# undistro/trivy

Hardware: AMD Instinct MI355X
Metric: GB/s secret-scanned (whole node) at 1/2/4/8 MI355X; findings bit-exact vs CPU (higher is better)
Workload: dtype u8

## Files before the change

include/tsg_debug.h:

```cpp
#ifndef TSG_DEBUG_H
#define TSG_DEBUG_H
#include <stdint.h>
#ifdef __cplusplus
extern "C" {
#endif

int tsg_regex_find_all(const char* pattern, const uint8_t* text, uint64_t n, int submatch,
                       const int64_t* windows, uint32_t n_windows, int64_t* out, uint64_t out_cap,
                       uint64_t* out_len, int32_t* num_cap);

void tsg_debug_regex_engine(int mode);
int tsg_debug_xform(int device, const uint8_t* raw, uint64_t n_bytes, const uint64_t* offsets, uint32_t n_files,
                    const uint8_t* kinds, uint8_t* out, uint64_t out_cap, uint64_t* xoff);
int tsg_debug_classify(int device, const uint8_t* raw, uint64_t n_bytes, const uint64_t* offsets, uint32_t n_files,
                       uint8_t* flags);
int tsg_debug_transform_census(int device, const uint8_t* raw, uint64_t n_bytes, const uint64_t* offsets,
                               uint32_t n_files, const uint8_t* kinds, uint8_t* mark_out);
int tsg_debug_gather_device(int device, const uint8_t* raw, uint64_t n_bytes, const uint64_t* src_off,
                            const uint64_t* dst_off, uint32_t n_files, uint8_t* out);
int tsg_regex_match(const char* pattern, const uint8_t* text, uint64_t n);

int64_t tsg_go_bytes_to_lower(const uint8_t* s, uint64_t n, uint8_t* out, uint64_t out_cap);

struct tsg_global;
typedef struct tsg_compiled tsg_compiled;
struct tsg_table_info;
typedef struct tsg_debug_rule_info {
  uint32_t nfa_words;
  uint32_t gate;
  uint32_t anchored;
  uint32_t has_regex;
  const uint64_t* nfa;
  const uint32_t* kw_ids;
  uint32_t n_kw;
} tsg_debug_rule_info;
int tsg_debug_compile(const struct tsg_global* g, tsg_compiled** out);
struct tsg_compile_options;
int tsg_debug_compile_ex(const struct tsg_global* g, const struct tsg_compile_options* opt, tsg_compiled** out,
                         uint32_t* out_calibrated);
void tsg_debug_compiled_free(tsg_compiled* c);
int tsg_debug_compiled_info(const tsg_compiled* c, struct tsg_table_info* out);
int tsg_debug_rule(const tsg_compiled* c, uint32_t i, tsg_debug_rule_info* out);
int tsg_debug_rule_gate_implied(const tsg_compiled* c, uint32_t i);
int tsg_debug_anchor(const tsg_compiled* c, uint32_t j, uint32_t* rule, uint32_t* lit_len,
                     int32_t* off_lo, int32_t* off_hi);
const char* tsg_debug_keyword(const tsg_compiled* c, uint32_t k);
const void* tsg_debug_anchor_req(const tsg_compiled* c, uint32_t j);
int tsg_debug_filter(const tsg_compiled* c, uint32_t* shape, const uint32_t** reach, const uint32_t** bucket_off,
                     const uint32_t** bucket_items, const void** items, uint32_t* n_items, const uint8_t** item_cls,
                     const uint32_t** classes, double* est_fp);
int tsg_debug_filter_ids(const tsg_compiled* c, const uint32_t** ids, uint32_t* n);
int tsg_debug_filter_core(const tsg_compiled* c, uint32_t out[4]);
const char* tsg_debug_rule_anchor(const tsg_compiled* c, uint32_t i);


int tsg_debug_pool_budget(void);

struct tsg_scanner;
int tsg_debug_scanner_engine(struct tsg_scanner* s, uint64_t out[4]);
int tsg_debug_filter_orform(const tsg_compiled* c, uint32_t out[1024]);

int tsg_debug_scanner_gpu_findings(struct tsg_scanner* s, int mode);

int tsg_debug_scanner_fetch(struct tsg_scanner* s, uint64_t stage_bytes, uint64_t direct_bytes);

int tsg_regex_find_all_bounded(const char* pattern, const uint8_t* text, uint64_t true_len, uint64_t lo, uint64_t hi,
                               int submatch, const int64_t* windows, uint32_t n_windows, int64_t* out,
                               uint64_t out_cap, uint64_t* out_len, int32_t* num_cap, int32_t* hit_limit);
int tsg_debug_fetch_windows_plan(const uint64_t* offsets, uint32_t n_files, const void* cands, uint64_t n_cands,
                                 const uint32_t* rule_max_len, uint32_t n_rules, const uint32_t* opts, uint64_t* runs,
                                 uint64_t runs_cap, uint64_t* n_runs, uint64_t* views, uint64_t views_cap,
                                 uint64_t* n_views, uint64_t totals[4]);
int tsg_debug_fetch_windows_device(int device, const uint8_t* arena, uint64_t n_bytes, const uint64_t* offsets,
                                   uint32_t n_files, const void* cands, uint64_t n_cands, uint32_t cand_cap,
                                   const uint32_t* rule_max_len, uint32_t n_rules, const uint32_t* opts,
                                   uint64_t stage_bytes, uint8_t* packed, uint64_t packed_cap, uint64_t counters[4]);

struct tsg_batch;
struct tsg_result;
struct tsg_fetch_window_stats;
int tsg_debug_sparse_tail(const struct tsg_global* g, const struct tsg_batch* batch, const void* cands,
                          uint64_t n_cands, const uint32_t* opts, struct tsg_result** out,
                          struct tsg_fetch_window_stats* window_stats);

int tsg_debug_sure_allow(const char* const* patterns, uint32_t n_patterns, const uint8_t* paths, const uint64_t* off,
                         uint32_t n_paths, uint8_t* sure, uint8_t* has_form);
int tsg_debug_result_skip(const struct tsg_result* r, uint64_t out[6]);
int tsg_debug_result_k0(const struct tsg_result* r, double* ms_k0);

typedef struct tsg_debug_stage_dump {
  uint32_t struct_size;
  uint32_t kw_words;
  uint32_t counters[16];
  uint32_t caps[3];
  uint32_t reserved_;
  uint64_t* hits;        uint64_t hits_cap, n_hits;
  uint32_t* kw;          uint64_t kw_cap, n_kw;
  uint32_t* flags;       uint64_t flags_cap, n_flags;
  uint16_t* nl;          uint64_t nl_cap, n_nl;
  uint32_t* chunk_file;  uint64_t chunk_file_cap, n_chunk_file;
  uint32_t* recs;        uint64_t recs_cap, n_recs;
  void* cands;           uint64_t cands_cap, n_cands;
} tsg_debug_stage_dump;
int tsg_debug_engine_stages(const tsg_compiled* c, int device, const uint8_t* arena, uint64_t n_bytes,
                            const uint64_t* offsets, uint32_t n_files, const uint8_t tail[64],
                            tsg_debug_stage_dump* out);
int tsg_debug_engine_stages_skip(const tsg_compiled* c, int device, const uint8_t* arena, uint64_t n_bytes,
                                 const uint64_t* offsets, uint32_t n_files, const uint8_t tail[64],
                                 const uint8_t* skip, tsg_debug_stage_dump* out);
int tsg_debug_scan_grow(const uint32_t counters[16], const uint32_t fs_counters[6], uint32_t caps[7]);

int tsg_debug_tar_headers(int device, const void* dev_tar, uint64_t n_bytes, uint64_t capacity, uint32_t grid_cap,
                          void* records_out, uint64_t* count_out, double* ms_out);
void tsg_debug_set_tar_capacity(uint64_t records);
struct tsg_analyzer;
struct tsg_tar_index;
struct tsg_device_tar_stats;
int tsg_debug_index_tar_records(struct tsg_analyzer* a, const uint8_t* host_tar, uint64_t n_bytes,
                                const void* records, uint64_t n_records, struct tsg_tar_index** out,
                                struct tsg_device_tar_stats* st);
int tsg_debug_tar_chain(int device, const void* dev_tar, uint64_t n_bytes, uint32_t segment_blocks, uint32_t grid_cap,
                        void* records_out, uint64_t rec_cap, uint64_t* n_records, uint8_t* names_out,
                        uint64_t name_cap, uint64_t* name_bytes, uint64_t* stop_out, uint64_t* candidates_out);
int tsg_debug_tar_walk_last_fallback(const struct tsg_analyzer* a);
int tsg_debug_index_tar_entries(struct tsg_analyzer* a, const void* records, uint64_t n_records, const uint8_t* names,
                                uint64_t name_bytes, const uint64_t* stop, uint64_t n_bytes,
                                uint64_t candidates_given, struct tsg_tar_index** out,
                                struct tsg_device_tar_stats* st);
int tsg_debug_tar_batch_plan(const struct tsg_tar_index* ix, uint32_t first, uint32_t count, const uint8_t* flags,
                             uint64_t* base, uint64_t* offs, uint8_t* kinds, uint8_t* binary);

const char* tsg_last_error(void);

#ifdef __cplusplus
}
#endif
#endif
```

trivy_amd/csrc/capi_debug.cpp:

```cpp
#include "tsg_debug.h"

#include <algorithm>
#include <atomic>
#include <cstring>
#include <memory>
#include <string>
#include <vector>

#include "capi_internal.h"
#include "census.h"
#include "classify.h"
#include "fetch_host.h"
#include "fetch_windows.h"
#include "filter.h"
#include "goregex.h"
#include "k1_orform.h"
#include "parallel.h"
#include "xform.h"

namespace tsg {
extern std::atomic<int> g_regex_engine;
thread_local std::string g_last_error;
void SetError(const std::string& e) { g_last_error = e; }
}
// ... 439 lines not shown

int tsg_debug_engine_stages(const tsg_compiled* c, int device, const uint8_t* arena, uint64_t n_bytes,
                            const uint64_t* offsets, uint32_t n_files, const uint8_t tail[64],
                            tsg_debug_stage_dump* out) {
  return tsg_debug_engine_stages_skip(c, device, arena, n_bytes, offsets, n_files, tail, nullptr, out);
}

int tsg_debug_engine_stages_skip(const tsg_compiled* c, int device, const uint8_t* arena, uint64_t n_bytes,
                                 const uint64_t* offsets, uint32_t n_files, const uint8_t tail[64],
                                 const uint8_t* skip, tsg_debug_stage_dump* out) {
  if (!c || !offsets || !tail || !out || (n_bytes && !arena)) {
    tsg::SetError("tsg_debug_engine_stages: NULL argument");
    return -2;
  }
  if (out->struct_size != sizeof(tsg_debug_stage_dump)) {
    tsg::SetError("tsg_debug_engine_stages: unknown tsg_debug_stage_dump.struct_size");
    return -2;
  }
  if (!WinArgsOk("tsg_debug_engine_stages", offsets, n_files, nullptr)) return -2;
  if (offsets[n_files] != n_bytes) {
    tsg::SetError("tsg_debug_engine_stages: offsets must end at n_bytes");
    return -2;
  }
  void *d_arena = nullptr, *d_off = nullptr, *d_skip = nullptr;
  hipError_t e = hipSetDevice(device);
  auto ok = [&](hipError_t r) {
    if (e == hipSuccess) e = r;
    return e == hipSuccess;
  };
  tsg::StageDump d;
  std::string run_err;
  if (ok(e) && ok(hipMalloc(&d_arena, n_bytes + 64)) && ok(hipMalloc(&d_off, (size_t(n_files) + 1) * 8)) &&
      ok(hipMemcpy(static_cast<uint8_t*>(d_arena) + n_bytes, tail, 64, hipMemcpyHostToDevice)) &&
      (n_bytes == 0 || ok(hipMemcpy(d_arena, arena, n_bytes, hipMemcpyHostToDevice))) &&
      ok(hipMemcpy(d_off, offsets, (size_t(n_files) + 1) * 8, hipMemcpyHostToDevice)) &&
      (!skip || n_files == 0 ||
       (ok(hipMalloc(&d_skip, n_files)) && ok(hipMemcpy(d_skip, skip, n_files, hipMemcpyHostToDevice))))) {
    std::unique_ptr<tsg::GpuEngine> eng(new tsg::GpuEngine(c->cr, device));
    std::vector<tsg::Candidate> cands;
    tsg::SkipIn sk;
    sk.d_skip = static_cast<const uint8_t*>(d_skip);
    if (!eng->ok() || !eng->Run(static_cast<const uint8_t*>(d_arena), n_bytes, static_cast<const uint64_t*>(d_off),
                                n_files, &cands, nullptr, nullptr, d_skip ? &sk : nullptr, &d))
      run_err = eng->error().empty() ? "engine failed" : eng->error();
  }
  for (void* p : {d_arena, d_off, d_skip})
    if (p) (void)hipFree(p);
  if (e != hipSuccess || !run_err.empty()) {
    tsg::SetError(std::string("tsg_debug_engine_stages: ") + (e != hipSuccess ? hipGetErrorString(e) : run_err.c_str()));
    return -1;
  }
  out->kw_words = d.kw_words;
  static_assert(sizeof(out->counters) == tsg::kScanCtrBytes, "tsg_debug_stage_dump hands out the scan counters whole");
  std::memcpy(out->counters, d.counters, sizeof(out->counters));
  out->caps[0] = d.hit_cap;
  out->caps[1] = d.rec_cap;
  out->caps[2] = d.cand_cap;
  auto put = [](void* dst, uint64_t cap, uint64_t* n, const void* src, size_t count, size_t rec) {
    *n = count;
    const size_t k = size_t(std::min<uint64_t>(cap, count));
    if (dst && k) std::memcpy(dst, src, k * rec);
  };
  std::vector<uint64_t> hits(3 * d.hits.size());
  for (size_t i = 0; i < d.hits.size(); i++) {
    hits[3 * i] = d.hits[i].file;
    hits[3 * i + 1] = d.hits[i].end;
    hits[3 * i + 2] = d.hits[i].aid;
  }
  put(out->hits, out->hits_cap, &out->n_hits, hits.data(), d.hits.size(), 24);
  put(out->kw, out->kw_cap, &out->n_kw, d.kw.data(), d.kw.size(), 4);
  put(out->flags, out->flags_cap, &out->n_flags, d.flags.data(), d.flags.size(), 4);
  put(out->nl, out->nl_cap, &out->n_nl, d.nl.data(), d.nl.size(), 2);
  put(out->chunk_file, out->chunk_file_cap, &out->n_chunk_file, d.chunk_file.data(), d.chunk_file.size(), 4);
  put(out->recs, out->recs_cap, &out->n_recs, d.recs.data(), d.recs.size(), 4);
  put(out->cands, out->cands_cap, &out->n_cands, d.cands.data(), d.cands.size(), sizeof(tsg::Candidate));
  return 0;
}

int tsg_debug_scan_grow(const uint32_t* counters, const uint32_t* fs_counters, uint32_t caps[7]) {
  static_assert(tsg::kScanCtrWords == 16 && tsg::kNFsCtr == 6, "the sizes tsg_debug.h states");
  tsg::ScanCaps c;
  uint32_t* const field[7] = {&c.hit, &c.cand, &c.rec, &c.fold, &c.fs_pair, &c.fs_task, &c.fs_task_bytes};
  for (int i = 0; i < 7; i++) *field[i] = caps[i];
  const int which = tsg::GrowOverflowed(counters, fs_counters, &c);
  for (int i = 0; i < 7; i++) caps[i] = *field[i];
  return which;
}

int tsg_debug_pool_budget(void) { return tsg::PoolBudget(); }

int tsg_debug_filter_core(const tsg_compiled* c, uint32_t out[4]) {
  const auto* f = c->cr.filter.get();
  if (!f) return -1;
  const uint32_t n_groups = uint32_t(f->core.size() / 256);
  std::vector<std::vector<uint64_t>> cols;
  for (uint32_t b = 0; b < 256; b++) {
    std::vector<uint64_t> col(n_groups);
    for (uint32_t g = 0; g < n_groups; g++) col[g] = f->core[size_t(g) * 256 + b];
    if (std::find(cols.begin(), cols.end(), col) == cols.end()) cols.push_back(std::move(col));
  }
  uint32_t most = 0;
  for (uint32_t b = 0; b + 1 < f->bucket_groups.size(); b++) most = std::max(most, f->bucket_groups[b + 1] - f->bucket_groups[b]);
  out[0] = n_groups;
  out[1] = uint32_t(cols.size());
  out[2] = most;
  out[3] = uint32_t(f->hash_keys.size());
  return 0;
}

int tsg_debug_filter_orform(const tsg_compiled* c, uint32_t out[1024]) {
  const auto* f = c->cr.filter.get();
  if (!f || f->n_buckets != 16 || f->n_words != 4 || f->window > 6 || f->reach.size() != 256 * 4) return -1;
  for (uint32_t b = 0; b < 256; b++) tsg::OrFormRow(&f->reach[size_t(b) * 4], out + size_t(b) * 4);
  return 0;
}

int tsg_debug_sure_allow(const char* const* patterns, uint32_t n_patterns, const uint8_t* paths, const uint64_t* off,
                         uint32_t n_paths, uint8_t* sure, uint8_t* has_form) {
  std::vector<std::unique_ptr<tsg::Regex>> own;
  std::vector<const tsg::Regex*> res;
  for (uint32_t i = 0; i < n_patterns; i++) {
    std::string err;
    own.push_back(tsg::Regex::Compile(patterns[i], &err));
    if (!own.back()) {
      tsg::SetError(err);
      return -1;
    }
    res.push_back(own.back().get());
  }
  tsg::SureTable t;
  std::vector<uint8_t> form;
  tsg::SureTableOf(res, &t, &form);
  if (has_form && n_patterns) std::memcpy(has_form, form.data(), n_patterns);
  for (uint32_t i = 0; i < n_paths; i++) sure[i] = tsg::SureAllowHost(t, paths + off[i], off[i + 1] - off[i]) ? 1 : 0;
  return 0;
}

int tsg_debug_result_skip(const struct tsg_result* r, uint64_t out[6]) {
  if (!r) return -1;
  std::memcpy(out, r->skip, sizeof(r->skip));
  return 0;
}

int tsg_debug_result_k0(const struct tsg_result* r, double* ms_k0) {
  if (!r || !ms_k0) return -1;
  *ms_k0 = r->ms_k0;
  return 0;
}
}
```

trivy_amd/csrc/capi_scanner.cpp:

```cpp
#include <pthread.h>
#include <condition_variable>
#include <cstring>
#include <deque>
#include <mutex>
#include <thread>
#include <memory>
#include <string>

#include "capi_internal.h"
#include "filter.h"
#include "scanner.h"
#include "tsg_debug.h"
#include "tsg_scanner.h"

namespace {
class ResultReaper {
 public:
  static ResultReaper& Get() {
    static ResultReaper r;
    return r;
  }
  void Push(tsg_result* r) {
    if (!r) return;
    {
// ... 600 lines not shown

int tsg_debug_rule(const tsg_compiled* c, uint32_t i, tsg_debug_rule_info* out) {
  if (i >= c->cr.rules.size()) return -1;
  const auto& r = c->cr.rules[i];
  out->nfa_words = r.nfa_words;
  out->gate = r.gate;
  out->anchored = r.anchored;
  out->has_regex = r.has_regex;
  out->nfa = c->cr.nfa.data() + r.nfa_off;
  out->kw_ids = c->cr.rule_kw.data() + r.kw_off;
  out->n_kw = r.kw_cnt;
  return 0;
}

int tsg_debug_rule_gate_implied(const tsg_compiled* c, uint32_t i) {
  if (i >= c->cr.rules.size()) return -1;
  return c->cr.rules[i].kw_match_implied ? 1 : 0;
}

int tsg_debug_anchor(const tsg_compiled* c, uint32_t j, uint32_t* rule, uint32_t* lit_len, int32_t* off_lo,
                     int32_t* off_hi) {
  if (j >= c->cr.anchors.size()) return -1;
  const auto& a = c->cr.anchors[j];
  *rule = a.rule;
  *lit_len = a.lit_len;
  *off_lo = a.off_lo;
  *off_hi = a.off_hi;
  return 0;
}

int tsg_debug_filter(const tsg_compiled* c, uint32_t* shape, const uint32_t** reach, const uint32_t** bucket_off,
                     const uint32_t** bucket_items, const void** items, uint32_t* n_items, const uint8_t** item_cls,
                     const uint32_t** classes, double* est_fp) {
  const auto* f = c->cr.filter.get();
  if (!f) return -1;
  shape[0] = f->n_buckets;
  shape[1] = f->window;
  shape[2] = f->n_words;
  *reach = f->reach.data();
  *bucket_off = f->bucket_off.data();
  *bucket_items = f->bucket_items.data();
  *items = f->items.data();
  *n_items = uint32_t(f->items.size());
  *item_cls = f->item_cls.data();
  *classes = f->classes.data();
  *est_fp = f->est_fp;
  return 0;
}

int tsg_debug_filter_ids(const tsg_compiled* c, const uint32_t** ids, uint32_t* n) {
  const auto* f = c->cr.filter.get();
  if (!f) return -1;
  *ids = f->item_ids.data();
  *n = uint32_t(f->item_ids.size());
  return 0;
}

const char* tsg_debug_rule_anchor(const tsg_compiled* c, uint32_t i) {
  const auto& d = c->cr.rule_anchor_desc;
  return i < d.size() ? d[i].c_str() : nullptr;
}

const void* tsg_debug_anchor_req(const tsg_compiled* c, uint32_t j) {
  return j < c->cr.anchor_req.size() ? &c->cr.anchor_req[j] : nullptr;
}

const char* tsg_debug_keyword(const tsg_compiled* c, uint32_t k) {
  return k < c->cr.keywords.size() ? c->cr.keywords[k].c_str() : nullptr;
}

int tsg_debug_scanner_engine(tsg_scanner* s, uint64_t out[4]) {
  out[0] = out[1] = out[2] = out[3] = 0;
  if (!s || !s->s || s->s->n_engines() == 0) return -1;
  for (size_t i = 0; i < s->s->n_engines(); i++) {
    const tsg::GpuEngine::HostMemInfo m = s->s->engine_at(i)->host_mem_info();
    out[0] += m.retired_pending;
    out[1] += m.retired_freed;
    out[2] = std::max<uint64_t>(out[2], m.cand_cap);
    out[3] += m.slot_bytes;
  }
  return 0;
}

int tsg_scanner_set_fetch_options(tsg_scanner* s, const tsg_fetch_options* opt) {
  if (!s || !s->s || !opt) {
    tsg::SetError("tsg_scanner_set_fetch_options: NULL argument");
    return -1;
  }
  if (opt->struct_size != TSG_FETCH_OPTIONS_SIZE_V1) {
    tsg::SetError("tsg_scanner_set_fetch_options: tsg_fetch_options.struct_size " + std::to_string(opt->struct_size) +
                  " is not a size this library knows (v1 = " + std::to_string(TSG_FETCH_OPTIONS_SIZE_V1) + ")");
    return -1;
  }
  if (opt->mode > TSG_FETCH_WINDOWS) {
    tsg::SetError("tsg_scanner_set_fetch_options: mode " + std::to_string(opt->mode) +
                  " (0 = files, 1 = windows are the modes)");
    return -1;
  }
  if (opt->back_bytes != 0 && opt->back_bytes < tsg::kFetchBackMin) {
    tsg::SetError("tsg_scanner_set_fetch_options: back_bytes " + std::to_string(opt->back_bytes) +
                  " is below 4 (the regex engine looks back one rune)");
    return -1;
  }
  tsg::FetchWinParams p;
  if (opt->back_bytes) p.back = opt->back_bytes;
  if (opt->fwd_bytes) p.fwd_bytes = opt->fwd_bytes;
  if (opt->fwd_cap) p.fwd_cap = opt->fwd_cap;
  if (opt->max_span) p.max_span = opt->max_span;
  s->s->SetFetchOptions(opt->mode == TSG_FETCH_WINDOWS, p);
  return 0;
}

int tsg_scanner_get_fetch_options(const tsg_scanner* s, tsg_fetch_options* out) {
  if (!s || !s->s || !out) {
    tsg::SetError("tsg_scanner_get_fetch_options: NULL argument");
    return -1;
  }
  if (out->struct_size != TSG_FETCH_OPTIONS_SIZE_V1) {
    tsg::SetError("tsg_scanner_get_fetch_options: tsg_fetch_options.struct_size " + std::to_string(out->struct_size) +
                  " is not a size this library knows (v1 = " + std::to_string(TSG_FETCH_OPTIONS_SIZE_V1) + ")");
    return -1;
  }
  tsg::FetchWinParams p;
  out->mode = s->s->GetFetchOptions(&p) ? TSG_FETCH_WINDOWS : TSG_FETCH_FILES;
  out->back_bytes = p.back;
  out->fwd_bytes = p.fwd_bytes;
  out->fwd_cap = p.fwd_cap;
  out->max_span = p.max_span;
  return 0;
}

int tsg_result_fetch_window_stats(const tsg_result* r, tsg_fetch_window_stats* out) {
  if (!r || !out) {
    tsg::SetError("tsg_result_fetch_window_stats: NULL argument");
    return -1;
  }
  if (out->struct_size != TSG_FETCH_WINDOW_STATS_SIZE_V1) {
    tsg::SetError("tsg_result_fetch_window_stats: tsg_fetch_window_stats.struct_size " +
                  std::to_string(out->struct_size) + " is not a size this library knows (v1 = " +
                  std::to_string(TSG_FETCH_WINDOW_STATS_SIZE_V1) + ")");
    return -1;
  }
  out->mode_used = r->win.mode_used;
  out->granules = r->win.granules;
  out->runs = r->win.runs;
  out->window_bytes = r->win.window_bytes;
  out->sparse_files = r->win.sparse_files;
  out->whole_files = r->win.whole_files;
  out->fallback_files = r->win.fallback_files;
  out->fallback_bytes = r->win.fallback_bytes;
  out->ms_fallback = r->win.ms_fallback;
  return 0;
}

int tsg_scanner_set_resident_transform(tsg_scanner* s, uint32_t mode) {
  if (!s || !s->s) {
    tsg::SetError("tsg_scanner_set_resident_transform: NULL argument");
    return -1;
  }
  if (mode > TSG_RESIDENT_SPLIT) {
    tsg::SetError("tsg_scanner_set_resident_transform: mode " + std::to_string(mode) +
                  " (0 = chunked, 1 = split are the modes)");
    return -1;
  }
  s->s->SetResidentTransform(mode);
  return 0;
// ... 46 lines not shown
```

trivy_amd/csrc/engine.h:

```cpp
#pragma once
#include <hip/hip_runtime.h>

#include <cstdint>
#include <atomic>
#include <condition_variable>
#include <deque>
#include <memory>
#include <string>
#include <mutex>
#include <thread>
#include <vector>

#include "fetch_layout.h"
#include "rules.h"
#include "scan_layout.h"

namespace tsg {

constexpr uint32_t kChunk = 1024;

constexpr uint32_t kCandGateOpen = 1;
constexpr uint32_t kCandFoldFile = 2;
constexpr uint32_t kCandGateValid = 4;
constexpr uint32_t kCandDrop = 8;
// ... 83 lines not shown
  hipEvent_t ev_fs = nullptr;
  hipEvent_t ev_k0[2] = {};
  bool Create();
  void Destroy();
};

struct SkipIn {
  const uint8_t* d_skip = nullptr;
  hipEvent_t ready = nullptr;
  bool drop_marked = false;
};

class GpuEngine {
 public:
  GpuEngine(const CompiledRules& cr, int device);
  ~GpuEngine();
  bool ok() const { return err_.empty(); }
  const std::string& error() const { return err_; }
  int device() const { return device_; }
  hipStream_t stream() const { return stream_; }

  bool Run(const uint8_t* d_arena, uint64_t n_bytes, const uint64_t* d_offsets, uint32_t n_files,
           std::vector<Candidate>* cands, BatchStats* st, FetchOut* fetch = nullptr, const SkipIn* skip = nullptr,
           StageDump* dump = nullptr);
  bool FetchFiles(const uint8_t* d_arena, const uint64_t* d_offsets, uint32_t n_files,
                  const std::vector<uint8_t>& want, FetchOut* out);

  bool RunHost(const uint8_t* h_arena, uint64_t n_bytes, const uint64_t* h_offsets, uint32_t n_files,
               std::vector<Candidate>* cands, BatchStats* st, const uint8_t* kinds, TailOut* tail,
               std::mutex* dev_mu, std::string* err, const uint8_t* gather_base = nullptr,
               const uint64_t* gather_src = nullptr, const uint8_t* d_src = nullptr);

  struct Ticket {
    int slot = -1;
    uint32_t cand_copy = 0;
  };
  bool Enqueue(const uint8_t* d_arena, uint64_t n_bytes, const uint64_t* d_offsets, uint32_t n_files, Ticket* t,
               std::string* err, FetchOut* fetch = nullptr, const SkipIn* skip = nullptr);
  bool Collect(Ticket* t, std::vector<Candidate>* cands, BatchStats* st, bool* rerun, std::string* err,
               FetchOut* fetch = nullptr);

  void SetFetchSizes(uint64_t stage_bytes, uint64_t direct_bytes);
  void* TakeFetchBuf(size_t need, size_t* cap);
  void GiveFetchBuf(void* p, size_t cap);

 private:
  bool Ensure(void** p, size_t* cap, size_t need);
  struct WorkSet {
    void* chunk_file = nullptr; size_t cap_chunk_file = 0;
    void* keep_bits = nullptr; size_t cap_keep_bits = 0;
    void* runs = nullptr; size_t cap_runs = 0;
    uint32_t* skip_info = nullptr;
    void* kw = nullptr; size_t cap_kw = 0;
    void* flags = nullptr; size_t cap_flags = 0;
    void* cands = nullptr; size_t cap_cands = 0;
    uint32_t* counters = nullptr;
    uint32_t* fs_ctr = nullptr;
    hipEvent_t free_ev = nullptr, k0_done = nullptr;
    bool free_rec = false, k0_rec = false;
  };
  static constexpr int kSets = 2;
  WorkSet sets_[kSets];
  uint32_t set_turn_ = 0;
  hipStream_t aux_stream_ = nullptr;
  hipStream_t rb_stream_ = nullptr;
  bool overlap_k0_ = true, readback_stream_ = true;
  hipEvent_t k2_done_ = nullptr;
  bool k2_rec_ = false;
  struct KernelArgs;
  bool EnsureSets(uint64_t n_chunks, uint32_t n_files, uint64_t f_tiles, bool skip);
  bool EnqueuePhase(const uint8_t* d_arena, uint64_t n_bytes, const uint64_t* d_offsets, uint32_t n_files,
                    uint64_t n_chunks, WorkSet& W, bool k0_aux, PhaseEvents& E, const SkipIn* skip = nullptr);
  void InitCaps(uint64_t n_bytes);
  struct Slot {
    PhaseEvents ev;
    hipEvent_t done = nullptr;
    hipEvent_t fin = nullptr, rb_done = nullptr;
    uint32_t* h_cnt = nullptr;
    uint32_t* h_skip = nullptr;
    bool has_skip = false;
    Candidate* h_cands = nullptr;
    size_t h_cap = 0;
    bool busy = false, has_fs = false;
    uint64_t n_bytes = 0;
    uint32_t n_files = 0;
    bool has_fetch = false;
    hipEvent_t ev_f[2] = {};
    void* h_fctr = nullptr;
    void* lease = nullptr;
    size_t lease_cap = 0;
    uint64_t fetch_copy = 0;
    uint64_t stage = 0, direct = 0;
    bool win = false;
    FetchWinParams prm;
    const uint8_t* d_arena = nullptr;
  };
  static constexpr int kSlots = 4;
  std::atomic<uint32_t> cand_recent_{0};
  Slot slots_[kSlots];
  std::mutex slot_mu_;
  std::mutex dev_mu_;
  void RetireHost(void* p);
  void ReaperLoop();
  std::mutex reap_mu_;
  std::condition_variable reap_cv_;
  std::vector<void*> retired_host_;
  bool reap_stop_ = false;
  std::thread reaper_;
  std::atomic<uint64_t> retired_pending_{0}, retired_freed_{0};
  bool IssueFetch(const WorkSet& W, const uint8_t* d_arena, const uint64_t* d_offsets, uint32_t n_files,
                  const uint32_t* h_flags, uint64_t direct, uint64_t stage, uint64_t copy_bytes, uint8_t* h_dst,
                  void* h_ctr, hipEvent_t ev0);
  bool FetchNow(const uint8_t* d_arena, const uint64_t* d_offsets, uint32_t n_files, std::vector<uint8_t> want,
                bool upload_flags, FetchOut* out);
  void NoteFetch(uint64_t packed, uint64_t total);
  bool IssueFetchWin(const WorkSet& W, const uint8_t* d_arena, uint64_t n_bytes, const uint64_t* d_offsets,
                     uint32_t n_files, const FetchWinParams& prm, uint64_t stage, uint64_t copy_bytes, uint8_t* h_dst,
                     void* h_ctr, hipEvent_t ev0);
  bool FetchNowWin(const uint8_t* d_arena, uint64_t n_bytes, const uint64_t* d_offsets, uint32_t n_files,
                   const std::vector<Candidate>& cands, FetchOut* out);
  std::atomic<uint64_t> fetchw_stage_bytes_{uint64_t(256) << 20};
  std::atomic<uint64_t> fetchw_recent_packed_{0};
  void* d_wscratch_ = nullptr; size_t cap_wscratch_ = 0;
  uint32_t* d_rule_max_len_ = nullptr;
  std::vector<uint32_t> h_rule_max_len_;
  bool EnsureFetchStream();
  std::atomic<uint64_t> fetch_stage_bytes_{uint64_t(256) << 20}, fetch_direct_bytes_{uint64_t(8) << 20};
  std::atomic<uint64_t> fetch_recent_packed_{0}, fetch_recent_total_{0};
  hipStream_t fetch_stream_ = nullptr;
  hipEvent_t ev_packed_ = nullptr, ev_drained_ = nullptr, ev_run_f_[2] = {};
  void* d_fscratch_ = nullptr; size_t cap_fscratch_ = 0;
  void* d_fstage_ = nullptr; size_t cap_fstage_ = 0;
  void* d_fctr_ = nullptr;
  void* h_run_fctr_ = nullptr;
  void* h_fflags_ = nullptr; size_t cap_h_fflags_ = 0;
  std::unique_ptr<FetchPool> fetch_pool_;

 public:
  struct HostMemInfo {
    uint64_t retired_pending, retired_freed, cand_cap, slot_bytes;
  };
  HostMemInfo host_mem_info();

 private:
  bool Transform(int b, uint32_t nf, const uint8_t** arena, const uint64_t** offsets, uint64_t* n_bytes,
                 std::vector<uint64_t>* xoff, float* ms);
  bool GatherTail(const std::vector<Candidate>& part, uint32_t f0, uint32_t nf, const std::vector<uint64_t>& xoff,
                  const uint64_t* raw_off, const uint8_t* kinds, std::vector<uint64_t>* tail_len, TailOut* tail);
  void DumpItemDiag();
  bool DumpStages(const WorkSet& W, const uint32_t* cnt, uint64_t n_bytes, uint32_t n_files, StageDump* d);
  std::vector<uint8_t> h_items_kind_;
  std::vector<uint32_t> h_items_id_;
  std::string err_;
  int device_ = 0;
  hipStream_t stream_ = nullptr;
  PhaseEvents run_ev_;
  uint32_t diag_mode_ = 0, diag_confirm_ = 0;
  AnchorInfo* d_anchors_ = nullptr;
  RuleGpu* d_rules_ = nullptr;
  uint32_t* d_rule_kw_ = nullptr;
  uint64_t* d_nfa_ = nullptr;
  uint32_t* d_fullscan_rules_ = nullptr;
  uint32_t kw_words_ = 0, n_rules_ = 0, n_fullscan_rules_ = 0;
  std::vector<uint32_t> fullscan_rules_;
  uint32_t* d_reach_ = nullptr;
  uint64_t* d_core_ = nullptr;
  uint32_t* d_group_items_ = nullptr;
  uint32_t* d_bucket_groups_ = nullptr;
  void* d_ftabs_ = nullptr;
  void* d_fold_pairs_ = nullptr;
  void* d_fold_first_ = nullptr;
  uint32_t n_fold_pairs_k_ = 0, n_fold_pairs_s_ = 0, n_fold_cap_k_ = 0, n_fold_cap_s_ = 0;
  void* d_fold_idx_off_ = nullptr;
  void* d_fold_idx_items_ = nullptr;
  uint32_t n_fold_cap_k_idx_ = 0, n_fold_cap_s_idx_ = 0;
  void* d_kwfold_pairs_ = nullptr;
  uint32_t n_kwf_ri_ = 0, n_kwf_rk_ = 0, n_kwf_ci_ = 0, n_kwf_ck_ = 0;
  bool kw_fold_ = false;
  uint32_t ftabs_bytes_ = 0, ft_bucket_off_ = 0, ft_bucket_items_ = 0, ft_items_ = 0;
  uint32_t ft_item_ids_ = 0, ft_item_cls_ = 0, ft_classes_ = 0, ft_luts_ = 0;
  uint32_t ftabs_fold_bytes_ = 0, ft_cmap_ = 0, ft_ccore_ = 0, ft_gitems_ = 0, ft_bgroups_ = 0, n_core_cls_ = 0;
  uint32_t ft_hkeys_ = 0, ft_hitems_ = 0, hash_bits_ = 0, hash_buckets_ = 0;
  size_t c_lds_bytes_ = 0;
  bool lds_tabs_ = true;
  bool fold_stage_ = false;
  uint32_t fold_grid_ = 2048;
  bool c_stage_classes_ = false;
  size_t fold_stage_bytes_ = 0;
  uint32_t n_fclasses_ = 0;
  void* d_recs_ = nullptr; size_t cap_recs_ = 0;
  uint32_t n_fitems_ = 0;
  void* d_nl_ = nullptr; size_t cap_nl_ = 0;
  uint32_t* h_run_skip_ = nullptr;
  uint32_t k1_grid_cap_ = 0;
  void NoteSkip(const uint32_t* info, BatchStats* st) const;
  void* d_hits_ = nullptr; size_t cap_hits_ = 0;
  void* d_folds_ = nullptr; size_t cap_folds_ = 0;
  hipStream_t copy_stream_ = nullptr;
  static constexpr int kNStage = 4;
  struct HostCall;
  struct StageJob {
    uint64_t slot;
    HostCall* call;
    uint32_t f0, f1;
  };
  bool CopyChunk(const StageJob& j, std::string* err);
  void CopierLoop();
  std::mutex ring_mu_;
  std::condition_variable ring_cv_;
  std::deque<StageJob> ring_jobs_;
  uint64_t ring_next_ = 0, ring_turn_ = 0, ring_copied_ = 0;
  bool stage_ok_[kNStage] = {};
  std::string stage_err_[kNStage];
  bool ring_stop_ = false;
  std::thread copier_;
  hipEvent_t ev_copied_[kNStage] = {}, ev_h2d_[2] = {};
  void* d_stage_[kNStage] = {}; size_t cap_stage_[kNStage] = {};
  void* d_stage_off_[kNStage] = {}; size_t cap_stage_off_[kNStage] = {};
  uint64_t* h_off_[kNStage] = {}; size_t cap_h_off_[kNStage] = {};
  uint64_t* h_xoff_ = nullptr; size_t cap_h_xoff_ = 0;
  uint32_t* h_run_cnt_ = nullptr;
  void* h_run_cands_ = nullptr; size_t cap_h_run_cands_ = 0;
  void* h_gup_ = nullptr; size_t cap_h_gup_ = 0;
  void* h_gbuf_ = nullptr; size_t cap_h_gbuf_ = 0;
  bool EnsureHost(void** p, size_t* cap, size_t need);
  void* d_kind_[kNStage] = {}; size_t cap_kind_[kNStage] = {};
  void* d_gsrc_[kNStage] = {}; size_t cap_gsrc_[kNStage] = {};
  void* h_gsrc_[kNStage] = {}; size_t cap_h_gsrc_[kNStage] = {};
  void* d_xlen_ = nullptr; size_t cap_xlen_ = 0;
  void* d_xoff_ = nullptr; size_t cap_xoff_ = 0;
  void* d_xscan_ = nullptr; size_t cap_xscan_ = 0;
  void* d_xf_ = nullptr; size_t cap_xf_ = 0;
  void* d_gfiles_ = nullptr; size_t cap_gfiles_ = 0;
  void* d_gdst_ = nullptr; size_t cap_gdst_ = 0;
  void* d_gbuf_ = nullptr; size_t cap_gbuf_ = 0;
  hipEvent_t ev_x_[2] = {};
  uint64_t chunk_bytes_ = uint64_t(1) << 30;
  ScanCaps caps_;
  uint32_t fs_chunk_ = 65536;
  void* d_fs_pairs_ = nullptr; size_t cap_fs_pairs_ = 0;
  void* d_fs_tasks_ = nullptr; size_t cap_fs_tasks_ = 0;
  void* d_fs_wave_ = nullptr; size_t cap_fs_wave_ = 0;
  hipEvent_t ev_sync_ = nullptr;
  bool blocking_sync_ = true;
  uint32_t verify_blocks_ = 4096;
  uint32_t finalize_blocks_ = 16384;
  hipError_t WaitStream();
  hipError_t WaitEvent(hipEvent_t ev);
  uint32_t* d_item_diag_ = nullptr;
  std::string item_diag_path_;
};

}
```

trivy_amd/csrc/engine.hip:

```cpp
#include <chrono>
#include <condition_variable>
#include <mutex>
#include <hip/hip_runtime.h>

#include <algorithm>
#include <cstdlib>
#include <cstdio>
#include <cstring>
#include <string>
#include <pthread.h>

#include <thread>
#include <type_traits>

#include "engine.h"
#include "census.h"
#include "fetch.h"
#include "fetch_host.h"
#include "fetch_windows.h"
#include "xform.h"
#include "filter.h"
#include "k1_orform.h"

namespace tsg {
// ... 622 lines not shown
#endif
constexpr int kCThreads = TSG_C_THREADS;
#ifndef TSG_C_THREADS_G
#define TSG_C_THREADS_G 256
#endif
constexpr int kCThreadsG = TSG_C_THREADS_G;
template <bool kLdsTabs>
constexpr int ConfirmThreads() { return kLdsTabs ? kCThreads : kCThreadsG; }

struct FoldSite {
  uint64_t x;
  uint32_t f;
  uint32_t len;
};

__device__ __forceinline__ uint32_t wave_slot(uint32_t* ctr) {
  const uint64_t m = __ballot(1);
  const uint32_t leader = uint32_t(__ffsll(static_cast<unsigned long long>(m)) - 1);
  const uint32_t rank = __builtin_amdgcn_mbcnt_hi(uint32_t(m >> 32), __builtin_amdgcn_mbcnt_lo(uint32_t(m), 0u));
  uint32_t base = 0;
  if (rank == 0) base = atomicAdd(ctr, uint32_t(__popcll(m)));
  base = __shfl(base, int(leader));
  return base + rank;
}

#ifndef TSG_C_HITS
#define TSG_C_HITS 96
#endif
constexpr uint32_t kCWaveHits = TSG_C_HITS;

constexpr uint32_t kHitAidBits = 24;
__device__ __forceinline__ uint32_t hit_aid_word(uint32_t aid, uint64_t end) {
  return aid | (uint32_t(end >> 32) << kHitAidBits);
}
__host__ __device__ __forceinline__ void hit_unpack(const uint32_t* h, uint32_t* f, uint64_t* end, uint32_t* aid) {
  *f = h[0];
  *end = uint64_t(h[1]) | (uint64_t(h[2] >> kHitAidBits) << 32);
  *aid = h[2] & ((1u << kHitAidBits) - 1u);
}

__device__ __forceinline__ void stage_hit(uint32_t* hbuf, uint32_t* hcnt, uint32_t* hits, uint32_t cap,
                                          uint32_t* counters, uint32_t f, uint64_t end, uint32_t aid) {
  const uint32_t k = atomicAdd(hcnt, 1u);
  if (k < kCWaveHits) {
    hbuf[3 * k + 0] = f;
    hbuf[3 * k + 1] = uint32_t(end);
    hbuf[3 * k + 2] = hit_aid_word(aid, end);
    return;
  }
  const uint32_t g = atomicAdd(&counters[kCtHits], 1u);
  if (g < cap) {
    hits[3ull * g + 0] = f;
    hits[3ull * g + 1] = uint32_t(end);
    hits[3ull * g + 2] = hit_aid_word(aid, end);
  } else {
    counters[kCtHitOvf] = 1;
  }
}

__device__ __forceinline__ void flush_staged(uint32_t* hbuf, uint32_t* hcnt, uint32_t* hits, uint32_t cap,
                                             uint32_t* counters, uint32_t lane) {
  wave_sync();
  const uint32_t n_all = __builtin_amdgcn_readfirstlane(*hcnt);
  const uint32_t n = n_all < kCWaveHits ? n_all : kCWaveHits;
  if (n) {
    uint32_t base = 0;
    if (lane == 0) base = atomicAdd(&counters[kCtHits], n);
    base = __builtin_amdgcn_readfirstlane(base);
    for (uint32_t i = lane; i < n; i += 64) {
      if (base + i < cap) {
        hits[3ull * (base + i) + 0] = hbuf[3 * i + 0];
        hits[3ull * (base + i) + 1] = hbuf[3 * i + 1];
        hits[3ull * (base + i) + 2] = hbuf[3 * i + 2];
      } else {
        counters[kCtHitOvf] = 1;
      }
    }
  }
  wave_sync();
  if (lane == 0) *hcnt = 0;
  wave_sync();
}

__device__ __forceinline__ void put_hit(uint32_t* hits, uint32_t cap, uint32_t* counters, uint32_t f, uint64_t end,
                                        uint32_t aid) {
  const uint32_t g = wave_slot(&counters[kCtHits]);
  if (g < cap) {
    hits[3ull * g + 0] = f;
    hits[3ull * g + 1] = uint32_t(end);
    hits[3ull * g + 2] = hit_aid_word(aid, end);
  } else {
    counters[kCtHitOvf] = 1;
  }
}
__device__ __forceinline__ bool follow_lut_pass(const FollowLut& L, const uint32_t* X, int64_t avail) {
  const uint32_t n0 = L.n[0], n1 = L.n[1];
  if (n0 == 0) return true;
  const int64_t span0 = int64_t(L.hi[0]) + n0, span1 = n1 ? int64_t(L.hi[1]) + n1 : 0;
  const int64_t lim = avail < (span0 > span1 ? span0 : span1) ? avail : (span0 > span1 ? span0 : span1);
  uint32_t nonascii = 0;
#pragma unroll
  for (int j = 0; j < 13; j++) {
    const int64_t v = lim - 4 * j;
    const uint32_t vm = v >= 4 ? ~0u : (v <= 0 ? 0u : (1u << (8 * uint32_t(v))) - 1u);
    nonascii |= X[j] & vm;
  }
  if (nonascii & 0x80808080u) return true;
  uint32_t t[4], h[2];
  __builtin_memcpy(t, L.lo_tab, 16);
  __builtin_memcpy(h, L.hi_tab, 8);
  uint32_t M[13];
#pragma unroll
  for (int j = 0; j < 13; j++) {
    const uint32_t lo = X[j] & 0x0F0F0F0Fu, hi = (X[j] >> 4) & 0x07070707u;
    const uint32_t sel = lo & 0x07070707u;
    const uint32_t a0 = __builtin_amdgcn_perm(t[1], t[0], sel), a1 = __builtin_amdgcn_perm(t[3], t[2], sel);
    const uint32_t m8 = ((lo >> 3) & 0x01010101u) * 0xFFu;
    M[j] = ((a0 & ~m8) | (a1 & m8)) & __builtin_amdgcn_perm(h[1], h[0], hi);
  }
  auto interval = [&](int r, uint32_t n) -> uint64_t {
    int64_t a = L.lo[r], b = L.hi[r];
    if (avail - int64_t(n) < b) b = avail - int64_t(n);
    if (b < a) return 0;
    const uint64_t upto = b >= 63 ? ~uint64_t(0) : (uint64_t(1) << (b + 1)) - 1;
    return upto & ~((uint64_t(1) << a) - 1);
  };
  const uint64_t R0 = interval(0, n0), R1 = n1 ? interval(1, n1) : 0;
  uint32_t f0 = 0, f1 = 0;
#pragma unroll
  for (int j = 0; j < 12; j++) {
    const uint32_t y1 = __builtin_amdgcn_alignbyte(M[j + 1], M[j], 1);
    const uint32_t y2 = __builtin_amdgcn_alignbyte(M[j + 1], M[j], 2);
    const uint32_t y3 = __builtin_amdgcn_alignbyte(M[j + 1], M[j], 3);
    const uint32_t Z = M[j] & (y1 >> 1) & (y2 >> 2) & (y3 >> 3);
    const uint32_t s0 = ((uint32_t(R0 >> (4 * j)) & 0xFu) * 0x00204081u) & 0x01010101u;
    const uint32_t s1 = ((uint32_t(R1 >> (4 * j)) & 0xFu) * 0x00204081u) & 0x01010101u;
    f0 |= Z & s0;
    f1 |= Z & (s1 << 4);
  }
  return f0 != 0 && (n1 == 0 || f1 != 0);
}

__device__ __forceinline__ void follow_words(const uint32_t* w, uint32_t s, uint32_t* X) {
  uint32_t R[14];
#pragma unroll
  for (int j = 0; j < 14; j++) R[j] = w[j];
#pragma unroll
  for (int j = 0; j < 13; j++) X[j] = __builtin_amdgcn_alignbyte(R[j + 1], R[j], s & 3);
}

#ifndef TSG_C_WIN
#define TSG_C_WIN 48
#endif
constexpr int kCWin = TSG_C_WIN;

struct ConfirmParams {
  const uint8_t* arena;
  uint64_t n_bytes;
  const uint64_t* off;
  const uint32_t* chunk_file;
  const uint16_t* nl;
  const uint32_t* reach;
  const void* tabs;
  uint32_t tabs_bytes, t_bucket_off, t_bucket_items, t_items, t_item_ids, t_item_cls, t_classes;
  const AnchorInfo* anchors;
  const RuleGpu* rules;
  const uint64_t* nfa;
  const uint32_t* recs;
  uint32_t rec_cap;
  uint32_t* flags;
  uint32_t* counters;
  uint32_t* hits;
  uint32_t hit_cap;
  FoldSite* folds;
  uint32_t fold_cap;
  uint32_t diag;
  uint32_t* kwbits;
  uint32_t kw_words;
  const uint64_t* core;
  const uint32_t* group_items;
  const uint32_t* bucket_groups;
  uint32_t* item_diag;
  uint32_t t_luts;
  uint32_t t_cmap, t_ccore, t_gitems, t_bgroups, n_cls;
  uint32_t t_hkeys, t_hitems, hash_bits, hash_buckets;
  uint32_t n_classes_lds;
};

constexpr int kNfaReject = 0, kNfaAccept = 1, kNfaUndecided = 2;
template <int W>
__device__ int nfa_run_abs(const uint8_t* __restrict arena, uint64_t fs, int64_t len, int64_t start, int64_t inj_hi,
                           const uint64_t* __restrict tab, int64_t max_steps) {
  uint64_t O[W], Lp[W], F[W], D[W];
#pragma unroll
  for (int w = 0; w < W; w++) {
    O[w] = tab[w];
    Lp[w] = tab[W + w];
    F[w] = tab[2 * W + w];
    D[w] = 0;
  }
  const uint64_t* B = tab + 3 * W;
  uint4 buf = make_uint4(0, 0, 0, 0);
  uint64_t buf_at = ~uint64_t(0);
  const int64_t stop = len - start > max_steps ? start + max_steps : len;
  for (int64_t pos = start; pos < stop; pos++) {
    const uint64_t abs = fs + uint64_t(pos);
    if ((abs & ~uint64_t(15)) != buf_at) {
      buf_at = abs & ~uint64_t(15);
      buf = load16(arena + buf_at);
    }
    const uint32_t b = (word_of(buf, uint32_t(abs >> 2) & 3) >> ((abs & 3) * 8)) & 0xFFu;
    uint64_t carry = pos <= inj_hi ? 1 : 0;
    uint64_t T[W];
#pragma unroll
    for (int w = 0; w < W; w++) {
      T[w] = (D[w] << 1) | carry | (D[w] & Lp[w]);
      carry = D[w] >> 63;
    }
    uint64_t c = 0;
#pragma unroll
    for (int w = 0; w < W; w++) {
      uint64_t x = T[w] & O[w];
      uint64_t s1 = O[w] + x;
      uint64_t c1 = s1 < O[w];
      uint64_t s2 = s1 + c;
      uint64_t c2 = s2 < s1;
      T[w] |= s2 ^ O[w];
      c = c1 | c2;
    }
    const uint64_t* Bb = B + size_t(b) * W;
    const bool keep = (b & 0xC0u) == 0x80u;
    uint64_t acc = 0, alive = 0;
#pragma unroll
    for (int w = 0; w < W; w++) {
      uint64_t nd = (T[w] & Bb[w]) | (keep ? D[w] : 0);
      D[w] = nd;
      acc |= nd & F[w];
      alive |= nd;
    }
    if (acc) return kNfaAccept;
    if (!alive && pos >= inj_hi) return kNfaReject;
  }
  return stop < len ? kNfaUndecided : kNfaReject;
}

__device__ int nfa_dispatch_abs(int words, const uint8_t* arena, uint64_t fs, int64_t len, int64_t start,
                                int64_t inj_hi, const uint64_t* tab, int64_t max_steps = INT64_MAX) {
  switch (words) {
    case 1: return nfa_run_abs<1>(arena, fs, len, start, inj_hi, tab, max_steps);
    case 2: return nfa_run_abs<2>(arena, fs, len, start, inj_hi, tab, max_steps);
    case 3: return nfa_run_abs<3>(arena, fs, len, start, inj_hi, tab, max_steps);
    default: return nfa_run_abs<4>(arena, fs, len, start, inj_hi, tab, max_steps);
  }
}

__device__ __forceinline__ void put_candidate(Candidate* cands, uint32_t cap, uint32_t* counters, uint32_t f,
                                              uint32_t r, int64_t wlo, int64_t whi) {
  const uint32_t k = atomicAdd(&counters[kCtCands], 1u);
  if (k < cap) {
    Candidate c;
    c.file = f;
    c.rule = r;
    c.wlo = wlo;
    c.whi = whi;
    c.nl_before = -1;
    c.flags = 0;
    c.nl_back[0] = c.nl_back[1] = c.nl_back[2] = kNlUnknown;
    c.nl_fwd[0] = c.nl_fwd[1] = c.nl_fwd[2] = kNlUnknown;
    c.pad_ = 0;
    cands[k] = c;
  } else {
    counters[kCtCandOvf] = 1;
  }
}

__device__ int64_t count_nl_range(const uint8_t* arena, uint64_t a, uint64_t b) {
  int64_t n = 0;
  for (uint64_t blk = a & ~uint64_t(15); blk < b; blk += 16) {
    const uint4 v = load16(arena + blk);
#pragma unroll
    for (uint32_t q = 0; q < 4; q++) {
      const uint64_t wa = blk + 4 * q;
      const uint32_t lo = a > wa ? uint32_t(a - wa < 4 ? a - wa : 4) : 0u;
      const uint32_t hi = b < wa + 4 ? (b > wa ? uint32_t(b - wa) : 0u) : 4u;
      if (hi <= lo) continue;
      const uint32_t mhi = hi == 4 ? ~0u : (1u << (8 * hi)) - 1u;
      const uint32_t mlo = ~((1u << (8 * lo)) - 1u);
      n += nl_count4(word_of(v, q) & mhi & mlo);
    }
  }
  return n;
}

__device__ int64_t count_nl_abs(const uint8_t* arena, const uint16_t* nl, uint64_t a, uint64_t b) {
  const uint64_t ca = (a + kChunk - 1) / kChunk, cb = b / kChunk;
  if (ca >= cb) return count_nl_range(arena, a, b);
  int64_t n = count_nl_range(arena, a, ca * kChunk) + count_nl_range(arena, cb * kChunk, b);
  for (uint64_t c = ca; c < cb; c++) n += nl[c];
  return n;
}

#ifndef TSG_C_Q1
#define TSG_C_Q1 128
#endif
#ifndef TSG_C_Q2
#define TSG_C_Q2 96
#endif
constexpr uint32_t kCQ1 = TSG_C_Q1;
constexpr uint32_t kCQ2 = TSG_C_Q2;
constexpr size_t ConfirmFixedLds(int t) {
  return 4096 + size_t(t) * (kCWin + 8) + size_t(t / 64) * (kCQ1 + kCQ2) * 4 +
         size_t(t / 64) * kCWaveHits * 12 + size_t(t / 64) * 16;
}

template <bool kLdsTabs>
#ifndef TSG_C_MINW
#define TSG_C_MINW 4
#endif
__global__ __launch_bounds__(ConfirmThreads<kLdsTabs>(), TSG_C_MINW) void confirm_kernel(ConfirmParams P) {
  extern __shared__ __attribute__((aligned(16))) uint8_t smem[];
  constexpr int kCThreads = ConfirmThreads<kLdsTabs>();
  constexpr uint32_t kWaves = kCThreads / 64;
  uint8_t* s_reach = smem;
  uint8_t* s_win = smem + 4096;
  uint64_t* s_base = reinterpret_cast<uint64_t*>(s_win + kCThreads * kCWin);
  uint32_t* s_q1 = reinterpret_cast<uint32_t*>(s_base + kCThreads);
  uint32_t* s_q2 = s_q1 + kWaves * kCQ1;
  uint32_t* s_hbuf = s_q2 + kWaves * kCQ2;
  uint32_t* s_cnt = s_hbuf + kWaves * kCWaveHits * 3;
  uint8_t* s_tabs = reinterpret_cast<uint8_t*>(s_cnt + kWaves * 4);
  const int tid = threadIdx.x;
  load_reach_lds(s_reach, P.reach, tid, blockDim.x);
  if (kLdsTabs) {
    const uint4* t = reinterpret_cast<const uint4*>(P.tabs);
    uint4* d = reinterpret_cast<uint4*>(s_tabs);
    for (uint32_t i = tid; i < P.tabs_bytes / 16; i += blockDim.x) d[i] = t[i];
  }
  const uint8_t* tabs = kLdsTabs ? s_tabs : static_cast<const uint8_t*>(P.tabs);
  const uint32_t lane = tid & 63, wave = tid >> 6;
  uint32_t* cnt = s_cnt + wave * 4;
  if (lane < 4) cnt[lane] = 0;
  __syncthreads();
  const FilterItemGpu* items = reinterpret_cast<const FilterItemGpu*>(tabs + P.t_items);
  const uint32_t* item_ids = reinterpret_cast<const uint32_t*>(tabs + P.t_item_ids);
  const uint8_t* item_cls = tabs + P.t_item_cls;
  const uint32_t* classes = reinterpret_cast<const uint32_t*>(tabs + P.t_classes);
  if (!kLdsTabs && P.n_classes_lds) {
    const uint4* c = reinterpret_cast<const uint4*>(static_cast<const uint8_t*>(P.tabs) + P.t_classes);
    for (uint32_t i = tid; i < P.n_classes_lds * 2; i += blockDim.x) reinterpret_cast<uint4*>(s_tabs)[i] = c[i];
    __syncthreads();
    classes = reinterpret_cast<const uint32_t*>(s_tabs);
  }
  uint8_t* wwin = s_win + wave * 64 * kCWin;
  uint64_t* wbase = s_base + wave * 64;
  uint32_t* q1 = s_q1 + wave * kCQ1;
  uint32_t* q2 = s_q2 + wave * kCQ2;
  uint32_t* hbuf = s_hbuf + wave * kCWaveHits * 3;
  const uint32_t n_recs = P.counters[kCtRecs] < P.rec_cap ? P.counters[kCtRecs] : P.rec_cap;
  uint32_t n_anchor = 0;
  auto check_item = [&](uint32_t l, uint32_t k, uint32_t ix, uint32_t full) {
    const FilterItemGpu it = items[ix];
    const uint64_t base = wbase[l];
    const int64_t start = int64_t(base + k) + 1 - int64_t(it.back);
    if (start < 0 || uint64_t(start) + it.n > P.n_bytes) return;
    const uint32_t core_lo = full ? uint32_t(it.back) : (it.back > 8 ? it.back - 8u : 0u);
    const uint64_t cw0 = base >= 16 ? base - 16 : 0;
    const uint8_t* cwin = wwin + l * kCWin;
    auto sets_ok = [&](uint32_t q0, uint32_t q1) {
      for (uint32_t q = q0; q < q1; q++) {
        if (q >= core_lo && q < it.back) continue;
        const uint64_t pos = uint64_t(start) + q;
        const uint32_t bt = pos - cw0 < uint64_t(kCWin) ? uint32_t(cwin[pos - cw0]) : uint32_t(P.arena[pos]);
        const uint32_t c = item_cls[it.cls_off + q];
        if (!((classes[c * 8 + (bt >> 5)] >> (bt & 31)) & 1u)) return false;
      }
      return true;
    };
    const uint32_t check_to = it.lit_end < it.n && (P.diag & 32) ? it.lit_end : it.n;
    if (!sets_ok(0, check_to)) return;
    if (P.diag & 16) return;
    const uint64_t s0 = uint64_t(start);
    uint32_t f = P.chunk_file[s0 / kChunk];
    uint64_t fs = P.off[f], fe = P.off[f + 1];
    while (s0 >= fe) {
      f++;
      fs = fe;
      fe = P.off[f + 1];
    }
    if (s0 < fs || s0 + it.n > fe) return;
    if (P.diag & 8) return;
    if (it.kind == kItemKeyword) {
      const uint32_t id = item_ids[it.ids_off];
      uint32_t* w = &P.kwbits[uint64_t(f) * P.kw_words + (id >> 5)];
      const uint32_t bit = 1u << (id & 31);
      if (!(__hip_atomic_load(w, __ATOMIC_RELAXED, __HIP_MEMORY_SCOPE_AGENT) & bit)) atomicOr(w, bit);
      return;
    }
    if (it.kind == kItemFold) {
      const uint32_t fl = item_ids[it.ids_off] == 2 ? 3u : 5u;
      if (atomicOr(&P.flags[f], fl) == 0) atomicAdd(&P.counters[kCtSpecial], 1u);
      const uint32_t q = atomicAdd(&P.counters[kCtFolds], 1u);
      if (q < P.fold_cap) P.folds[q] = FoldSite{s0, f, it.n};
      else P.counters[kCtFoldOvf] = 1;
      return;
    }
    if (P.item_diag) atomicAdd(&P.item_diag[2 * ix], 1u);
    const uint64_t lit_end = (s0 - fs) + it.lit_end;
    const uint64_t e = s0 + it.lit_end;
    const uint64_t w0 = wbase[l] >= 16 ? wbase[l] - 16 : 0;
    uint32_t X[13];
    bool have_x = false;
    int after = check_to < it.n ? -1 : 1;
    for (uint32_t d = 0; d < it.n_ids; d++) {
      const uint32_t aid = item_ids[it.ids_off + d];
      n_anchor++;
      const FollowLut lut = reinterpret_cast<const FollowLut*>(tabs + P.t_luts)[aid];
      if (lut.n[0] && e < P.n_bytes) {
        if (!have_x) {
          follow_words(reinterpret_cast<const uint32_t*>(P.arena + (e & ~uint64_t(3))), uint32_t(e), X);
          have_x = true;
        }
        if (!follow_lut_pass(lut, X, int64_t(fe - e))) continue;
      }
      if (after < 0) after = sets_ok(check_to, it.n) ? 1 : 0;
      if (!after) return;
      stage_hit(hbuf, &cnt[0], P.hits, P.hit_cap, P.counters, f, lit_end, aid);
    }
  };
  auto run_q2 = [&]() {
    wave_sync();
    const uint32_t n2 = __builtin_amdgcn_readfirstlane(cnt[2]);
    const uint32_t m2 = n2 < kCQ2 ? n2 : kCQ2;
    for (uint32_t c2 = 0; c2 < m2; c2 += 64) {
      if (c2 + lane < m2) {
        const uint32_t e = q2[c2 + lane];
        check_item(e & 63u, (e >> 6) & 15u, (e >> 10) & 0x1FFFFFu, e >> 31);
      }
      if (__builtin_amdgcn_readfirstlane(cnt[0]) >= 64) flush_staged(hbuf, &cnt[0], P.hits, P.hit_cap, P.counters, lane);
    }
    wave_sync();
    if (lane == 0) cnt[2] = 0;
    wave_sync();
  };
  auto do_fire = [&](uint32_t e) {
    const uint32_t l = e & 63u, k = (e >> 6) & 15u;
    uint32_t fm = e >> 10;
    const uint64_t base = wbase[l];
    uint32_t cb[8];
    const uint64_t cw0 = base >= 16 ? base - 16 : 0;
    const uint8_t* cwin = wwin + l * kCWin;
#pragma unroll
    for (int q = 0; q < 8; q++) {
      const int64_t pos = int64_t(base + k) - 7 + q;
      cb[q] = pos < 0 ? 0u : uint32_t(cwin[uint64_t(pos) - cw0]);
    }
    auto queue_item = [&](uint32_t ix, uint32_t full) {
      const uint32_t slot = atomicAdd(&cnt[2], 1u);
      if (slot < kCQ2) q2[slot] = l | (k << 6) | (ix << 10) | (full << 31);
      else check_item(l, k, ix, full);
    };
    if (fm & P.hash_buckets) {
      uint64_t key = 0;
#pragma unroll
      for (int q = 0; q < 6; q++) {
        const uint32_t b = cb[2 + q];
        key |= uint64_t(b - 'A' < 26u ? b + 32 : b) << (8 * q);
      }
      const uint64_t* hk = reinterpret_cast<const uint64_t*>(tabs + P.t_hkeys);
      const uint32_t* hi = reinterpret_cast<const uint32_t*>(tabs + P.t_hitems);
      const uint32_t mask = (1u << P.hash_bits) - 1;
      const uint64_t want = key | (uint64_t(1) << 63);
      for (uint32_t slot = WindowHash(key, P.hash_bits);; slot = (slot + 1) & mask) {
        const uint64_t kk = hk[slot];
        if (!kk) break;
        if (kk == want) queue_item(hi[slot], 1u);
      }
    }
    const uint32_t* bgroups = kLdsTabs ? reinterpret_cast<const uint32_t*>(tabs + P.t_bgroups) : P.bucket_groups;
    const uint32_t* gitems = kLdsTabs ? reinterpret_cast<const uint32_t*>(tabs + P.t_gitems) : P.group_items;
    if (kLdsTabs) {
#pragma unroll
      for (int q = 0; q < 8; q++) cb[q] = tabs[P.t_cmap + cb[q]];
    }
    while (fm) {
      const uint32_t j = __builtin_ctz(fm);
      fm &= fm - 1;
      for (uint32_t g = bgroups[j]; g < bgroups[j + 1]; g++) {
        const uint64_t* ct = kLdsTabs ? reinterpret_cast<const uint64_t*>(tabs + P.t_ccore) + size_t(g) * P.n_cls
                                      : P.core + size_t(g) * 256;
        uint64_t cm = ~uint64_t(0);
#pragma unroll
        for (int q = 0; q < 8; q++) cm &= ct[cb[q]] >> (8 * q);
        uint32_t im = uint32_t(cm) & 0xFFu;
        while (im) {
          const uint32_t gi = __builtin_ctz(im);
          im &= im - 1;
          queue_item(gitems[g * 8 + gi], 0u);
        }
      }
    }
  };
  const uint32_t stride = gridDim.x * blockDim.x;
  auto load_win = [&](uint32_t rec, bool valid, uint4* dst) {
    const uint64_t base = uint64_t(rec) * 16;
    const uint64_t w0 = base >= 16 ? base - 16 : 0;
#pragma unroll
    for (int q = 0; q < kCWin / 16; q++)
      dst[q] = valid && w0 + 16 * q + 16 <= P.n_bytes + 64 ? load16(P.arena + w0 + 16 * q) : make_uint4(0, 0, 0, 0);
  };
  const uint32_t r_first = blockIdx.x * blockDim.x + wave * 64 + lane;
  uint32_t rec_next = r_first < n_recs ? P.recs[r_first] : 0u;
  uint4 dwn[kCWin / 16];
  load_win(rec_next, r_first < n_recs, dwn);
  uint32_t rec_nn = r_first + stride < n_recs ? P.recs[r_first + stride] : 0u;
  for (uint32_t r0 = blockIdx.x * blockDim.x + wave * 64; r0 < n_recs; r0 += stride) {
    const uint32_t r = r0 + lane;
    const uint32_t rec = rec_next;
    uint4 dw[kCWin / 16];
#pragma unroll
    for (int q = 0; q < kCWin / 16; q++) dw[q] = dwn[q];
    rec_next = rec_nn;
    load_win(rec_next, r + stride < n_recs, dwn);
    rec_nn = r + 2 * stride < n_recs ? P.recs[r + 2 * stride] : 0u;
    uint32_t fire_e[4], n_fire = 0;
    if (r < n_recs) {
      const uint64_t base = uint64_t(rec) * 16;
      const uint4 d0 = dw[0], d1 = dw[1];
      uint4* wl = reinterpret_cast<uint4*>(wwin + lane * kCWin);
#pragma unroll
      for (int q = 0; q < kCWin / 16; q++) wl[q] = dw[q];
      wbase[lane] = base;
      const uint4 pv = base >= 16 ? d0 : make_uint4(0, 0, 0, 0);
      const uint4 v = base >= 16 ? d1 : d0;
      uint32_t st[kFWords] = {~0u, ~0u, ~0u, ~0u};
      auto rd1 = [&](uint32_t w, uint32_t k) {
        return *reinterpret_cast<const uint4*>(s_reach + (((w >> (8 * k)) & 0xFFu) << 4));
      };
#pragma unroll
      for (uint32_t k = 11; k < 16; k++) reach_apply(rd1(word_of(pv, k >> 2), k & 3), st);
#pragma unroll
      for (uint32_t k = 0; k < 16; k++) {
        reach_apply(rd1(word_of(v, k >> 2), k & 3), st);
        const uint32_t z = st[0] & st[1] & st[2] & st[3];
        if ((~z & 0x00F00000u) && !(P.diag & 4)) {
          uint32_t fm = 0;
#pragma unroll
          for (int w = 0; w < kFWords; w++) fm |= ((~st[w] >> 20) & 0xFu) << (4 * w);
          const uint32_t fe = lane | (k << 6) | (fm << 10);
          if (n_fire < 4) fire_e[n_fire] = fe;
          else do_fire(fe);
          n_fire++;
        }
      }
    }
    {
      const uint32_t mine = n_fire < 4 ? n_fire : 4u;
      uint32_t incl = mine;
#pragma unroll
      for (int x = 1; x < 64; x <<= 1) {
        const uint32_t t = __shfl_up(incl, x);
        if (lane >= uint32_t(x)) incl += t;
      }
      const uint32_t at = __builtin_amdgcn_readfirstlane(cnt[1]) + incl - mine;
      for (uint32_t i = 0; i < mine; i++) {
        if (at + i < kCQ1) q1[at + i] = fire_e[i];
        else do_fire(fire_e[i]);
      }
      wave_sync();
      if (lane == 63) cnt[1] = at + mine < kCQ1 ? at + mine : kCQ1;
    }
    wave_sync();
    const uint32_t n1 = __builtin_amdgcn_readfirstlane(cnt[1]);
    const uint32_t m1 = n1 < kCQ1 ? n1 : kCQ1;
    for (uint32_t c1 = 0; c1 < m1; c1 += 64) {
      if (c1 + lane < m1) do_fire(q1[c1 + lane]);
      const uint32_t n2 = __builtin_amdgcn_readfirstlane(cnt[2]);
      if (n2 >= 64 || (c1 + 64 >= m1 && n2 > 0)) run_q2();
    }
    wave_sync();
    if (lane == 0) cnt[1] = 0;
    if (__builtin_amdgcn_readfirstlane(cnt[0]) >= 64) flush_staged(hbuf, &cnt[0], P.hits, P.hit_cap, P.counters, lane);
    wave_sync();
  }
  flush_staged(hbuf, &cnt[0], P.hits, P.hit_cap, P.counters, lane);
#pragma unroll
  for (int x = 32; x >= 1; x >>= 1) n_anchor += __shfl_xor(n_anchor, x);
  if (lane == 0 && n_anchor) atomicAdd(&P.counters[kCtAnchorHits], n_anchor);
}

struct FoldPair {
  uint32_t item;
  uint16_t lo, hi;
};
constexpr int kFoldTaskStarts = 12;
struct FoldParams {
  const uint8_t* arena;
  const uint64_t* off;
  const void* tabs;
  uint32_t tabs_bytes, t_items, t_item_ids, t_item_cls, t_classes, n_items;
  const FoldPair* pairs;
  uint32_t n_pairs_k, n_pairs_s, n_cap_k, n_cap_s;
  const uint32_t* first;
  const uint32_t* idx_off;
  const uint32_t* idx_items;
  uint32_t n_cap_k_idx, n_cap_s_idx;
  const FoldSite* folds;
  uint32_t fold_cap;
  uint32_t* hits;
  uint32_t hit_cap;
  uint32_t* counters;
  uint32_t stage_items, n_classes;
  uint32_t diag;
};

constexpr int kFoldSpan = 3 * 48;
constexpr int kFoldIdxQ = 64;
constexpr int kFoldWin = 2 * kFoldSpan + 16;
constexpr int kFoldWaves = 4;

#ifndef TSG_FOLD_COOP_TASKS
#define TSG_FOLD_COOP_TASKS 512
#endif
#ifndef TSG_FOLD_WIDE_WPE
#define TSG_FOLD_WIDE_WPE 8
#endif
template <bool kLdsTabs, int kWaves = kFoldWaves>
__global__ __launch_bounds__(64 * kWaves) __attribute__((amdgpu_waves_per_eu(kWaves == 16 ? TSG_FOLD_WIDE_WPE : 1)))
void fold_kernel(FoldParams P) {
  extern __shared__ __attribute__((aligned(16))) uint8_t smem[];
  __shared__ uint8_t s_win[kWaves][kFoldWin];
  __shared__ uint32_t s_idx[kWaves][2][64];
  if (kLdsTabs) {
    const uint4* t = reinterpret_cast<const uint4*>(P.tabs);
    uint4* d = reinterpret_cast<uint4*>(smem);
    for (uint32_t i = threadIdx.x; i < P.tabs_bytes / 16; i += blockDim.x) d[i] = t[i];
    const uint4* f = reinterpret_cast<const uint4*>(P.first);
    uint4* df = reinterpret_cast<uint4*>(smem + P.tabs_bytes);
    for (uint32_t i = threadIdx.x; i < P.n_items * 2; i += blockDim.x) df[i] = f[i];
  } else if (P.stage_items) {
    const uint4* t = reinterpret_cast<const uint4*>(static_cast<const uint8_t*>(P.tabs) + P.t_items);
    uint4* d = reinterpret_cast<uint4*>(smem);
    for (uint32_t i = threadIdx.x; i < P.n_items; i += blockDim.x) d[i] = t[i];
    const uint4* c = reinterpret_cast<const uint4*>(static_cast<const uint8_t*>(P.tabs) + P.t_classes);
    uint4* dc = reinterpret_cast<uint4*>(smem + 16 * size_t(P.n_items));
    for (uint32_t i = threadIdx.x; i < P.n_classes * 2; i += blockDim.x) dc[i] = c[i];
  }
  __syncthreads();
  const uint8_t* tabs = kLdsTabs ? smem : static_cast<const uint8_t*>(P.tabs);
  const uint32_t* firsts = kLdsTabs ? reinterpret_cast<const uint32_t*>(smem + P.tabs_bytes) : P.first;
  const bool staged = !kLdsTabs && P.stage_items;
  const FilterItemGpu* items =
      staged ? reinterpret_cast<const FilterItemGpu*>(smem) : reinterpret_cast<const FilterItemGpu*>(tabs + P.t_items);
  const uint32_t* item_ids = reinterpret_cast<const uint32_t*>(tabs + P.t_item_ids);
  const uint8_t* item_cls = tabs + P.t_item_cls;
  const uint32_t* classes = staged ? reinterpret_cast<const uint32_t*>(smem + 16 * size_t(P.n_items))
                                   : reinterpret_cast<const uint32_t*>(tabs + P.t_classes);
  auto in_cls = [&](uint32_t c, uint32_t b) { return (classes[c * 8 + (b >> 5)] >> (b & 31)) & 1u; };
  const uint32_t lane = threadIdx.x & 63, wave = threadIdx.x >> 6;
  struct SiteCtx {
    uint64_t x, w0, w1, fs;
    uint32_t f;
    const uint8_t* wb;
  };
  auto try_start = [&](const SiteCtx& S, uint32_t ix, uint32_t back) {
    if (S.x < S.w0 + back) return;
    const FilterItemGpu it = items[ix];
    const uint32_t* first = firsts + 8ull * ix;
    const uint64_t st = S.x - back;
    const uint32_t b0 = S.wb[st - S.w0];
    if (!((first[b0 >> 5] >> (b0 & 31)) & 1u)) return;
// ... 758 lines not shown
        }
        found += __shfl(incl, 63);
        lo = ((lo >> 4) + 64) << 4;
      }
      if (lo >= fe)
        for (uint32_t r = found + lane; r < 3; r += 64) c.nl_fwd[r] = kNlNone;
    }
    if (lane == 0) c.flags = fl;
  }
}

template <typename T>
bool Upload(std::string* err, T** dst, const T* src, size_t n) {
  size_t bytes = std::max<size_t>(n * sizeof(T), 16);
  if (hipMalloc(dst, bytes + 16) != hipSuccess) {
    *err = "hipMalloc failed for tables";
    return false;
  }
  if (n && hipMemcpy(*dst, src, n * sizeof(T), hipMemcpyHostToDevice) != hipSuccess) {
    *err = "hipMemcpy failed for tables";
    return false;
  }
  return true;
}

}

GpuEngine::GpuEngine(const CompiledRules& cr, int device) : device_(device) {
  fetch_pool_.reset(new FetchPool(
      size_t(kSlots) + 2,
      [](size_t n) -> void* {
        void* p = nullptr;
        return hipHostMalloc(&p, n, hipHostMallocDefault) == hipSuccess ? p : nullptr;
      },
      [this](void* p) { RetireHost(p); }));
  if (hipSetDevice(device) != hipSuccess) {
    err_ = "hipSetDevice failed (no HIP device?)";
    return;
  }
  if (hipStreamCreateWithFlags(&stream_, hipStreamNonBlocking) != hipSuccess ||
      hipStreamCreateWithFlags(&copy_stream_, hipStreamNonBlocking) != hipSuccess) {
    err_ = "hipStreamCreate failed";
    return;
  }
  {
    if (const char* e = std::getenv("TSG_OVERLAP_K0")) overlap_k0_ = std::atoi(e) != 0;
    if (const char* e = std::getenv("TSG_READBACK_STREAM")) readback_stream_ = std::atoi(e) != 0;
    int lo = 0, hi = 0;
    if (hipDeviceGetStreamPriorityRange(&lo, &hi) != hipSuccess) lo = hi = 0;
    bool ok = hipStreamCreateWithPriority(&aux_stream_, hipStreamNonBlocking, hi) == hipSuccess &&
              hipStreamCreateWithFlags(&rb_stream_, hipStreamNonBlocking) == hipSuccess;
    for (WorkSet& W : sets_)
      ok = ok && hipEventCreateWithFlags(&W.free_ev, hipEventDisableTiming) == hipSuccess &&
           hipEventCreateWithFlags(&W.k0_done, hipEventDisableTiming) == hipSuccess;
    ok = ok && run_ev_.Create();
    ok = ok && hipEventCreateWithFlags(&k2_done_, hipEventDisableTiming) == hipSuccess;
    if (!ok) {
      err_ = "hipStreamCreate / hipEventCreate failed (K0 and read-back streams)";
      return;
    }
  }
  for (auto& e : ev_copied_) hipEventCreateWithFlags(&e, hipEventDisableTiming);
  for (auto& e : ev_h2d_) hipEventCreate(&e);
  for (auto& e : ev_x_) hipEventCreate(&e);
  if (const char* cm = std::getenv("TSG_INGEST_CHUNK_MB")) chunk_bytes_ = uint64_t(std::atoll(cm)) << 20;
  if (chunk_bytes_ < (uint64_t(1) << 20)) chunk_bytes_ = uint64_t(1) << 20;
  {
    const char* sm = std::getenv("TSG_FETCH_STAGE_MB");
    const char* dm = std::getenv("TSG_FETCH_DIRECT_MB");
    if (sm || dm)
      SetFetchSizes(sm ? uint64_t(std::max(1ll, std::atoll(sm))) << 20 : fetch_stage_bytes_.load(),
                    dm ? uint64_t(std::max(1ll, std::atoll(dm))) << 20 : fetch_direct_bytes_.load());
  }
  if (const char* dm = std::getenv("TSG_DIAG_SCAN")) diag_mode_ = uint32_t(std::atoi(dm));
  if (const char* dc = std::getenv("TSG_DIAG_CONFIRM")) diag_confirm_ = uint32_t(std::atoi(dc));
  if (const char* kg = std::getenv("TSG_DIAG_K1_GRID")) k1_grid_cap_ = uint32_t(std::max(0, std::atoi(kg)));
  if (const char* di = std::getenv("TSG_DIAG_ITEMS")) item_diag_path_ = di;
  if (const char* fc = std::getenv("TSG_FULLSCAN_CHUNK")) fs_chunk_ = uint32_t(std::atoi(fc));
  if (fs_chunk_ < 64) fs_chunk_ = 64;
  if (const char* tb = std::getenv("TSG_FS_TASK_BYTES")) caps_.fs_task_bytes = uint32_t(std::max(16, std::atoi(tb)));
  hipEventCreateWithFlags(&ev_sync_, hipEventBlockingSync | hipEventDisableTiming);
  if (const char* bs = std::getenv("TSG_BLOCKING_SYNC")) blocking_sync_ = std::atoi(bs) != 0;
  if (const char* vb = std::getenv("TSG_VERIFY_BLOCKS")) verify_blocks_ = uint32_t(std::max(1, std::atoi(vb)));
  if (const char* fb = std::getenv("TSG_FINALIZE_BLOCKS")) finalize_blocks_ = uint32_t(std::max(1, std::atoi(fb)));
  kw_words_ = std::max<uint32_t>(1, cr.kw_words());
  n_rules_ = uint32_t(cr.rules.size());
  for (uint32_t r = 0; r < n_rules_; r++)
    if (cr.rules[r].has_regex && !cr.rules[r].anchored) fullscan_rules_.push_back(r);
  n_fullscan_rules_ = uint32_t(fullscan_rules_.size());
  if (cr.anchors.size() >= (size_t(1) << kHitAidBits)) {
    err_ = "too many anchors for the hit records (>= 2^24)";
    return;
  }
  h_rule_max_len_.resize(cr.rules.size());
  for (size_t r = 0; r < cr.rules.size(); r++) h_rule_max_len_[r] = cr.rules[r].max_len;
  if (!Upload(&err_, &d_anchors_, cr.anchors.data(), cr.anchors.size()) ||
      !Upload(&err_, &d_rule_max_len_, h_rule_max_len_.data(), h_rule_max_len_.size()) ||
      !Upload(&err_, &d_rules_, cr.rules.data(), cr.rules.size()) ||
      !Upload(&err_, &d_rule_kw_, cr.rule_kw.data(), cr.rule_kw.size()) ||
      !Upload(&err_, &d_nfa_, cr.nfa.data(), cr.nfa.size()) ||
      !Upload(&err_, &d_fullscan_rules_, fullscan_rules_.data(), fullscan_rules_.size()))
    return;
  for (WorkSet& W : sets_)
    if (hipMalloc(&W.counters, kScanCtrBytes) != hipSuccess || hipMalloc(&W.fs_ctr, kScanCtrBytes) != hipSuccess) {
      err_ = "hipMalloc counters";
      return;
    }
  {
    const FilterTables* ft = cr.filter.get();
    if (!ft || ft->n_words != uint32_t(kFWords) || ft->window != uint32_t(kFWindow) || ft->nl_bucket != 15) {
      err_ = "prefilter shape not supported by the scan kernel (needs 16 buckets, window 6)";
      return;
    }
    if (!Upload(&err_, &d_reach_, ft->reach.data(), ft->reach.size()) ||
        !Upload(&err_, &d_core_, ft->core.data(), ft->core.size()) ||
        !Upload(&err_, &d_group_items_, ft->group_items.data(), ft->group_items.size()) ||
        !Upload(&err_, &d_bucket_groups_, ft->bucket_groups.data(), ft->bucket_groups.size()))
      return;
    auto pad = [](std::vector<uint8_t>& v) { v.resize((v.size() + 15) & ~size_t(15), 0); };
    std::vector<uint8_t> tb;
    auto put = [&](const void* src, size_t n) {
      size_t at = tb.size();
      tb.resize(at + n);
      if (n) std::memcpy(&tb[at], src, n);
      pad(tb);
      return uint32_t(at);
    };
    ft_bucket_off_ = put(ft->bucket_off.data(), ft->bucket_off.size() * 4);
    ft_bucket_items_ = put(ft->bucket_items.data(), ft->bucket_items.size() * 4);
    ft_items_ = put(ft->items.data(), ft->items.size() * sizeof(FilterItemGpu));
    ft_item_ids_ = put(ft->item_ids.data(), ft->item_ids.size() * 4);
    ft_item_cls_ = put(ft->item_cls.data(), ft->item_cls.size());
    ft_classes_ = put(ft->classes.data(), ft->classes.size() * 4);
    ft_luts_ = put(cr.anchor_req.data(), cr.anchor_req.size() * sizeof(FollowLut));
    if (tb.empty()) tb.assign(16, 0);
    ftabs_fold_bytes_ = uint32_t(tb.size());
    {
      const size_t n_groups = ft->bucket_groups.empty() ? 0 : ft->bucket_groups.back();
      std::vector<uint8_t> cmap(256, 0);
      std::vector<uint32_t> rep;
      for (uint32_t b = 0; b < 256; b++) {
        uint32_t c = 0;
        for (; c < rep.size(); c++) {
          bool same = true;
          for (size_t g = 0; g < n_groups && same; g++) same = ft->core[g * 256 + b] == ft->core[g * 256 + rep[c]];
          if (same) break;
        }
        if (c == rep.size()) rep.push_back(b);
        cmap[b] = uint8_t(c);
      }
      n_core_cls_ = uint32_t(rep.size());
      std::vector<uint64_t> cc(n_groups * rep.size());
      for (size_t g = 0; g < n_groups; g++)
        for (size_t c = 0; c < rep.size(); c++) cc[g * rep.size() + c] = ft->core[g * 256 + rep[c]];
      ft_cmap_ = put(cmap.data(), cmap.size());
      ft_ccore_ = put(cc.data(), cc.size() * sizeof(uint64_t));
      ft_gitems_ = put(ft->group_items.data(), ft->group_items.size() * 4);
      ft_bgroups_ = put(ft->bucket_groups.data(), ft->bucket_groups.size() * 4);
      ft_hkeys_ = put(ft->hash_keys.data(), ft->hash_keys.size() * 8);
      ft_hitems_ = put(ft->hash_items.data(), ft->hash_items.size() * 4);
      hash_bits_ = ft->hash_bits;
      hash_buckets_ = ft->hash_keys.empty() ? 0u : ft->hash_buckets;
    }
    ftabs_bytes_ = uint32_t(tb.size());
    n_fitems_ = uint32_t(ft->items.size());
    n_fclasses_ = uint32_t(ft->classes.size() / 8);
// ... 131 lines not shown
        }
        auto add = [&](std::vector<FoldPair>& v, int64_t lo, int64_t hi) {
          hi = std::min<int64_t>(hi, 0xFFFF);
          for (int64_t a = lo; a <= hi; a += kFoldTaskStarts)
            v.push_back({i, uint16_t(a), uint16_t(std::min<int64_t>(a + kFoldTaskStarts - 1, hi))});
        };
        if (ilo >= 0) add(ri, ilo, ihi);
        if (klo >= 0) add(rk, klo, khi);
      }
      n_kwf_ri_ = uint32_t(ri.size());
      n_kwf_rk_ = uint32_t(rk.size());
      n_kwf_ci_ = uint32_t(ci.size());
      n_kwf_ck_ = uint32_t(ck.size());
      ri.insert(ri.end(), rk.begin(), rk.end());
      ri.insert(ri.end(), ci.begin(), ci.end());
      ri.insert(ri.end(), ck.begin(), ck.end());
      if (ri.empty()) ri.push_back({0, 0, 0});
      uint8_t* dp = nullptr;
      if (!Upload(&err_, &dp, reinterpret_cast<const uint8_t*>(ri.data()), ri.size() * sizeof(FoldPair))) return;
      d_kwfold_pairs_ = dp;
      if (const char* e = std::getenv("TSG_KWFOLD")) kw_fold_ = kw_fold_ && std::atoi(e) != 0;
    }
    const size_t fixed = ConfirmFixedLds(kCThreads);
    size_t lds_max = 160 * 1024 * size_t(kCThreads) / 1024;
    if (const char* e = std::getenv("TSG_LDS_TABS_MAX")) lds_max = size_t(std::strtoull(e, nullptr, 10));
    size_t fold_static = kFoldWaves * kFoldWin;
    {
      hipFuncAttributes fa{};
      if (hipFuncGetAttributes(&fa, reinterpret_cast<const void*>(&fold_kernel<true>)) == hipSuccess)
        fold_static = std::max(fold_static, size_t(fa.sharedSizeBytes));
    }
    lds_tabs_ = fixed + ftabs_bytes_ <= lds_max && ftabs_fold_bytes_ + 32 * size_t(n_fitems_) + fold_static <= 64 * 1024;
    if (!item_diag_path_.empty() && hipMalloc(&d_item_diag_, 8 * std::max<size_t>(n_fitems_, 1)) != hipSuccess) {
      err_ = "hipMalloc item diag";
      return;
    }
    c_lds_bytes_ = lds_tabs_ ? fixed + ftabs_bytes_ : ConfirmFixedLds(kCThreadsG);
    {
      const char* sc = std::getenv("TSG_CONFIRM_STAGE_CLASSES");
      c_stage_classes_ = !lds_tabs_ && c_lds_bytes_ + 32 * size_t(n_fclasses_) <= 40 * 1024 && (!sc || std::atoi(sc) != 0);
      if (c_stage_classes_) c_lds_bytes_ += 32 * size_t(n_fclasses_);
    }
    if (std::getenv("TSG_ENGINE_DEBUG"))
      std::fprintf(stderr, "confirm LDS: fixed %zu + tables %u (fold prefix %u) = %zu B, limit %zu, %s tables, %d threads; "
                   "fold kernel static LDS %zu B\n",
                   fixed, ftabs_bytes_, ftabs_fold_bytes_, c_lds_bytes_, lds_max, lds_tabs_ ? "LDS" : "global",
                   lds_tabs_ ? kCThreads : kCThreadsG, fold_static);
    hipFuncSetAttribute(reinterpret_cast<const void*>(lds_tabs_ ? &confirm_kernel<true> : &confirm_kernel<false>),
                        hipFuncAttributeMaxDynamicSharedMemorySize, int(c_lds_bytes_));
    if (lds_tabs_)
      hipFuncSetAttribute(reinterpret_cast<const void*>(&fold_kernel<true>), hipFuncAttributeMaxDynamicSharedMemorySize,
                          int(ftabs_fold_bytes_ + 32 * n_fitems_));
    fold_stage_bytes_ = 16 * size_t(n_fitems_) + 32 * size_t(n_fclasses_);
    const char* fse = std::getenv("TSG_FOLD_STAGE");
    fold_stage_ = !lds_tabs_ && fold_stage_bytes_ <= 48 * 1024 && (!fse || std::atoi(fse) != 0);
    if (const char* fg = std::getenv("TSG_FOLD_GRID")) fold_grid_ = uint32_t(std::max(1, std::atoi(fg)));
    if (std::getenv("TSG_ENGINE_DEBUG"))
      std::fprintf(stderr, "fold: %u items, %u classes, staged %s (%zu B), %d waves per workgroup\n",
                   n_fitems_, n_fclasses_,
                   lds_tabs_ ? "(LDS tables)" : fold_stage_ ? "yes" : "no", fold_stage_bytes_,
                   fold_stage_ ? 16 : kFoldWaves);
    if (fold_stage_)
      hipFuncSetAttribute(reinterpret_cast<const void*>(&fold_kernel<false, 16>),
                          hipFuncAttributeMaxDynamicSharedMemorySize, int(fold_stage_bytes_));
  }
}

GpuEngine::~GpuEngine() {
  {
    std::lock_guard<std::mutex> g(ring_mu_);
    ring_stop_ = true;
  }
  ring_cv_.notify_all();
  if (copier_.joinable()) copier_.join();
  {
    std::lock_guard<std::mutex> g(reap_mu_);
    reap_stop_ = true;
  }
  reap_cv_.notify_all();
  if (reaper_.joinable()) reaper_.join();
  hipSetDevice(device_);
  void* ps[] = {d_item_diag_, d_fold_pairs_, d_kwfold_pairs_, d_fold_idx_off_, d_fold_idx_items_, d_fold_first_, d_reach_, d_core_, d_group_items_, d_bucket_groups_, d_ftabs_, d_folds_, d_recs_, d_anchors_,
                d_rules_, d_rule_kw_, d_nfa_, d_fullscan_rules_, d_nl_,
                d_hits_, d_fs_pairs_, d_fs_tasks_, d_fs_wave_, d_xlen_, d_xoff_, d_xscan_,
                d_xf_, d_gfiles_, d_gdst_, d_gbuf_};
  for (void* p : ps)
    if (p) hipFree(p);
  for (WorkSet& W : sets_) {
    for (void* p : {W.chunk_file, W.keep_bits, W.runs, static_cast<void*>(W.skip_info), W.kw, W.flags, W.cands,
                    static_cast<void*>(W.counters), static_cast<void*>(W.fs_ctr)})
      if (p) hipFree(p);
    if (W.free_ev) hipEventDestroy(W.free_ev);
    if (W.k0_done) hipEventDestroy(W.k0_done);
  }
  run_ev_.Destroy();
  if (k2_done_) hipEventDestroy(k2_done_);
  for (int b = 0; b < kNStage; b++)
  {
    for (void* p : {d_stage_[b], d_stage_off_[b], d_kind_[b], d_gsrc_[b]})
      if (p) hipFree(p);
    if (h_gsrc_[b]) hipHostFree(h_gsrc_[b]);
  }
  for (auto& e : ev_copied_)
    if (e) hipEventDestroy(e);
  if (ev_sync_) hipEventDestroy(ev_sync_);
  for (auto& S : slots_) {
    S.ev.Destroy();
    for (hipEvent_t e : {S.done, S.fin, S.rb_done})
      if (e) hipEventDestroy(e);
    if (S.h_cnt) hipHostFree(S.h_cnt);
    if (S.h_skip) hipHostFree(S.h_skip);
    if (S.h_cands) hipHostFree(S.h_cands);
    for (auto& e : S.ev_f)
      if (e) hipEventDestroy(e);
    if (S.h_fctr) hipHostFree(S.h_fctr);
    if (S.lease) hipHostFree(S.lease);
  }
  for (void* p : {d_fscratch_, d_fstage_, d_fctr_, d_wscratch_, static_cast<void*>(d_rule_max_len_)})
    if (p) hipFree(p);
  for (void* h : {h_run_fctr_, h_fflags_})
    if (h) hipHostFree(h);
  for (void* p : fetch_pool_->Drain()) hipHostFree(p);
  for (hipEvent_t e : {ev_packed_, ev_drained_, ev_run_f_[0], ev_run_f_[1]})
    if (e) hipEventDestroy(e);
  if (fetch_stream_) hipStreamDestroy(fetch_stream_);
  for (void* p : retired_host_) hipHostFree(p);
  for (auto& e : ev_h2d_)
    if (e) hipEventDestroy(e);
  for (auto& e : ev_x_)
    if (e) hipEventDestroy(e);
  for (auto* h : h_off_)
    if (h) hipHostFree(h);
  if (h_xoff_) hipHostFree(h_xoff_);
  for (void* h : {static_cast<void*>(h_run_cnt_), static_cast<void*>(h_run_skip_), h_run_cands_, h_gup_, h_gbuf_})
    if (h) hipHostFree(h);
  if (copy_stream_) hipStreamDestroy(copy_stream_);
  if (aux_stream_) hipStreamDestroy(aux_stream_);
  if (rb_stream_) hipStreamDestroy(rb_stream_);
  if (stream_) hipStreamDestroy(stream_);
}

bool GpuEngine::Ensure(void** p, size_t* cap, size_t need) {
  if (*p && *cap >= need) return true;
  if (*p) {
    HIP_OK(hipStreamSynchronize(aux_stream_));
    HIP_OK(hipStreamSynchronize(stream_));
    HIP_OK(hipStreamSynchronize(rb_stream_));
    if (fetch_stream_) HIP_OK(hipStreamSynchronize(fetch_stream_));
    hipFree(*p);
  }
  *p = nullptr;
  size_t n = std::max<size_t>(need + need / 8, 64);
  HIP_OK(hipMalloc(p, n));
  *cap = n;
  return true;
}

void GpuEngine::RetireHost(void* p) {
  {
    std::lock_guard<std::mutex> g(reap_mu_);
    retired_host_.push_back(p);
    retired_pending_.fetch_add(1);
    if (!reaper_.joinable()) reaper_ = std::thread([this] { ReaperLoop(); });
  }
  reap_cv_.notify_one();
}

void GpuEngine::ReaperLoop() {
  pthread_setname_np(pthread_self(), "tsg-hostfree");
  auto idle = [&] {
    {
      std::lock_guard<std::mutex> g(slot_mu_);
      for (const auto& S : slots_)
        if (S.busy) return false;
    }
    std::lock_guard<std::mutex> g(ring_mu_);
    return ring_turn_ == ring_next_;
  };
  std::unique_lock<std::mutex> lk(reap_mu_);
  for (;;) {
    reap_cv_.wait(lk, [&] { return reap_stop_ || !retired_host_.empty(); });
    if (reap_stop_) return;
    lk.unlock();
    while (!idle()) {
      lk.lock();
      const bool stop = reap_cv_.wait_for(lk, std::chrono::milliseconds(5), [&] { return reap_stop_; });
      lk.unlock();
      if (stop) return;
    }
    lk.lock();
    std::vector<void*> batch;
    batch.swap(retired_host_);
    lk.unlock();
    (void)hipSetDevice(device_);
    for (void* p : batch) {
      (void)hipHostFree(p);
      retired_pending_.fetch_sub(1);
      retired_freed_.fetch_add(1);
    }
    lk.lock();
  }
}

GpuEngine::HostMemInfo GpuEngine::host_mem_info() {
  HostMemInfo m{retired_pending_.load(), retired_freed_.load(), caps_.cand, 0};
  std::lock_guard<std::mutex> g(slot_mu_);
  for (const auto& S : slots_) m.slot_bytes += uint64_t(S.h_cap) * sizeof(Candidate);
  return m;
}

bool GpuEngine::EnsureHost(void** p, size_t* cap, size_t need) {
  if (*p && *cap >= need) return true;
  if (*p) hipHostFree(*p);
  *p = nullptr;
  *cap = 0;
  const size_t n = std::max<size_t>(need + need / 4, 4096);
  HIP_OK(hipHostMalloc(p, n, hipHostMallocDefault));
  *cap = n;
  return true;
}

static void RingLog(const char* what, uint64_t slot, uint64_t extra) {
  static const bool on = std::getenv("TSG_RING_DEBUG") && std::atoi(std::getenv("TSG_RING_DEBUG")) != 0;
  if (!on) return;
  static const auto t0 = std::chrono::steady_clock::now();
  const double ms = std::chrono::duration<double, std::milli>(std::chrono::steady_clock::now() - t0).count();
  std::fprintf(stderr, "ring %10.3f %-12s slot %llu %llu\n", ms, what, (unsigned long long)slot,
               (unsigned long long)extra);
}

struct GpuEngine::HostCall {
  const uint8_t* h_arena;
  const uint64_t* h_offsets;
  const uint8_t* kinds;
  const uint8_t* gather_dev = nullptr;
  const uint64_t* gather_src = nullptr;
  const uint8_t* d_src = nullptr;
  bool gather_device = false;
  bool cancelled = false;
  hipEvent_t ev0 = nullptr, ev1 = nullptr;
  bool ev0_recorded = false;
};

bool GpuEngine::CopyChunk(const StageJob& j, std::string* err) {
  const int b = int(j.slot % kNStage);
  const HostCall& c = *j.call;
  const uint64_t a = c.h_offsets[j.f0], e = c.h_offsets[j.f1];
  const uint32_t nf = j.f1 - j.f0;
  auto fail = [&](const char* what, hipError_t x) {
    *err = std::string(what) + ": " + hipGetErrorString(x);
    return false;
  };
  auto grow = [&](void** p, size_t* cap, size_t need, size_t floor) -> hipError_t {
    if (*p && *cap >= need) return hipSuccess;
    if (*p) hipFree(*p);
    *p = nullptr;
    *cap = 0;
    const size_t n = std::max(need + need / 2, floor);
    const hipError_t x = hipMalloc(p, n);
    if (x == hipSuccess) *cap = n;
    return x;
  };
  hipError_t x;
  if ((x = hipEventSynchronize(ev_copied_[b])) != hipSuccess) return fail("staging event", x);
  const size_t arena_need = (e - a) + 64;
  if ((x = grow(&d_stage_[b], &cap_stage_[b], arena_need,
                std::min<size_t>(chunk_bytes_, 4 * (e - a)) + 64)) != hipSuccess ||
      (x = grow(&d_stage_off_[b], &cap_stage_off_[b], (size_t(nf) + 1) * 8, 0)) != hipSuccess ||
      (c.kinds && (x = grow(&d_kind_[b], &cap_kind_[b], size_t(nf) + 1, 0)) != hipSuccess))
    return fail("staging hipMalloc", x);
  if (cap_h_off_[b] < size_t(nf) + 1) {
    if (h_off_[b]) hipHostFree(h_off_[b]);
    h_off_[b] = nullptr;
    cap_h_off_[b] = 0;
    const size_t n = size_t(nf) + 1 + (size_t(nf) + 1) / 2;
    if ((x = hipHostMalloc(reinterpret_cast<void**>(&h_off_[b]), n * 8, hipHostMallocDefault)) != hipSuccess)
      return fail("staging hipHostMalloc", x);
    cap_h_off_[b] = n;
  }
  for (uint32_t f = j.f0; f <= j.f1; f++) h_off_[b][f - j.f0] = c.h_offsets[f] - a;
  if (!c.ev0_recorded) {
    if ((x = hipEventRecord(c.ev0, copy_stream_)) != hipSuccess) return fail("hipEventRecord", x);
    j.call->ev0_recorded = true;
  }
  uint8_t* d = static_cast<uint8_t*>(d_stage_[b]);
  if (c.gather_dev) {
    std::vector<GatherItem> items;
    items.reserve(nf);
// ... 271 lines not shown
  HIP_OK(hipMemcpyAsync(h_xoff_, xo, (size_t(nf) + 1) * 8, hipMemcpyDeviceToHost, stream_));
  HIP_OK(hipMemcpyAsync(h_xoff_ + nf + 1, XformErrorPtr(raw_bytes, nf, d_xscan_), 4, hipMemcpyDeviceToHost, stream_));
  HIP_OK(hipEventRecord(ev_x_[1], stream_));
  HIP_OK(hipEventSynchronize(ev_x_[1]));
  const uint64_t total = h_xoff_[nf];
  if (const uint32_t xe = uint32_t(h_xoff_[nf + 1]); xe != 0 || total + 64 > cap_xf_) {
    err_ = "GPU pre-transform: output past its buffer (error word " + std::to_string(xe) + ", " +
           std::to_string(total) + " bytes)";
    return false;
  }
  if (XformOnePassOn()) HIP_OK(hipMemsetAsync(out + total, 0, 64, stream_));
  xoff->assign(h_xoff_, h_xoff_ + nf + 1);
  hipEventElapsedTime(ms, ev_x_[0], ev_x_[1]);
  *arena = out;
  *offsets = xo;
  *n_bytes = total;
  return true;
}

bool GpuEngine::GatherTail(const std::vector<Candidate>& part, uint32_t f0, uint32_t nf,
                           const std::vector<uint64_t>& xoff, const uint64_t* raw_off, const uint8_t* kinds,
                           std::vector<uint64_t>* tail_len, TailOut* tail) {
  std::vector<uint32_t> files;
  files.reserve(part.size());
  for (const auto& c : part)
    if (c.file < nf && (kinds[c.file] == 2 || xoff[c.file + 1] - xoff[c.file] != raw_off[c.file + 1] - raw_off[c.file]))
      files.push_back(c.file);
  std::sort(files.begin(), files.end());
  files.erase(std::unique(files.begin(), files.end()), files.end());
  for (uint32_t f : files) tail->raw[f0 + f] = 0;
  if (files.empty()) return true;
  std::vector<uint64_t> dst(files.size());
  uint64_t total = 0;
  for (size_t i = 0; i < files.size(); i++) {
    if (files[i] >= nf) {
      err_ = "candidate file outside its chunk";
      return false;
    }
    dst[i] = total;
    const uint64_t len = xoff[files[i] + 1] - xoff[files[i]];
    (*tail_len)[f0 + files[i]] = len;
    total += len;
  }
  if (!Ensure(&d_gfiles_, &cap_gfiles_, files.size() * 4) || !Ensure(&d_gdst_, &cap_gdst_, files.size() * 8) ||
      !Ensure(&d_gbuf_, &cap_gbuf_, total + 64))
    return false;
  const size_t up = files.size() * 12;
  if (!EnsureHost(&h_gup_, &cap_h_gup_, up) || !EnsureHost(&h_gbuf_, &cap_h_gbuf_, total + 1)) return false;
  uint8_t* hu = static_cast<uint8_t*>(h_gup_);
  std::memcpy(hu, dst.data(), dst.size() * 8);
  std::memcpy(hu + dst.size() * 8, files.data(), files.size() * 4);
  HIP_OK(hipMemcpyAsync(d_gdst_, hu, dst.size() * 8, hipMemcpyHostToDevice, stream_));
  HIP_OK(hipMemcpyAsync(d_gfiles_, hu + dst.size() * 8, files.size() * 4, hipMemcpyHostToDevice, stream_));
  HIP_OK(GatherFiles(static_cast<const uint8_t*>(d_xf_), static_cast<const uint64_t*>(d_xoff_),
                     static_cast<const uint32_t*>(d_gfiles_), static_cast<const uint64_t*>(d_gdst_),
                     uint32_t(files.size()), static_cast<uint8_t*>(d_gbuf_), stream_));
  HIP_OK(hipMemcpyAsync(h_gbuf_, d_gbuf_, total, hipMemcpyDeviceToHost, stream_));
  HIP_OK(WaitStream());
  const size_t at = tail->buf.size();
  tail->buf.resize(at + total);
  std::memcpy(tail->buf.data() + at, h_gbuf_, total);
  return true;
}

hipError_t GpuEngine::WaitEvent(hipEvent_t ev) {
  static const int poll_us = std::getenv("TSG_WAIT_POLL_US") ? std::atoi(std::getenv("TSG_WAIT_POLL_US")) : 200;
  if (poll_us <= 0) return hipEventSynchronize(ev);
  hipError_t e;
  while ((e = hipEventQuery(ev)) == hipErrorNotReady) std::this_thread::sleep_for(std::chrono::microseconds(poll_us));
  return e;
}

hipError_t GpuEngine::WaitStream() {
  if (!blocking_sync_ || !ev_sync_) return hipStreamSynchronize(stream_);
  hipError_t e = hipEventRecord(ev_sync_, stream_);
  return e != hipSuccess ? e : WaitEvent(ev_sync_);
}

void GpuEngine::InitCaps(uint64_t n_bytes) {
  if (caps_.hit == 0) caps_.hit = uint32_t(std::min<uint64_t>(std::max<uint64_t>(n_bytes / 512, 1 << 16), 1u << 28));
  if (caps_.cand == 0) caps_.cand = 1 << 16;
  if (caps_.rec == 0) caps_.rec = uint32_t(std::min<uint64_t>(std::max<uint64_t>(n_bytes / 128, 1 << 16), 1u << 30));
  if (caps_.fold == 0) caps_.fold = 1 << 16;
  if (caps_.fs_pair == 0) caps_.fs_pair = 1 << 14;
  if (caps_.fs_task == 0) caps_.fs_task = 1 << 16;
}

bool PhaseEvents::Create() {
  bool ok = hipEventCreate(&ev_fs) == hipSuccess;
  for (auto& e : ev) ok = ok && hipEventCreate(&e) == hipSuccess;
  for (auto& e : ev_k0) ok = ok && hipEventCreate(&e) == hipSuccess;
  return ok;
}

void PhaseEvents::Destroy() {
  for (hipEvent_t e : ev)
    if (e) (void)hipEventDestroy(e);
  for (hipEvent_t e : {ev_fs, ev_k0[0], ev_k0[1]})
    if (e) (void)hipEventDestroy(e);
}

static void NoteCounters(const uint32_t* cnt, BatchStats* st) {
  st->hits = cnt[kCtAnchorHits];
  st->follow_hits = cnt[kCtHits];
  st->special_files = cnt[kCtSpecial];
  st->flagged_blocks = cnt[kCtRecs];
  st->fullscan_tasks = cnt[kCtOpenPairs];
  st->fold_sites = cnt[kCtFolds];
  st->hit_overflow = cnt[kCtHitOvf] != 0;
  st->cand_overflow = cnt[kCtCandOvf] != 0;
}

static void NotePhaseTimes(const PhaseEvents& E, bool has_fs, BatchStats* st) {
  hipEventElapsedTime(&st->ms_scan, E.ev[kEvK1], E.ev[kEvK2]);
  hipEventElapsedTime(&st->ms_confirm, E.ev[kEvK2], E.ev[kEvFold]);
  hipEventElapsedTime(&st->ms_careful, E.ev[kEvFold], E.ev[kEvVerify]);
  hipEventElapsedTime(&st->ms_verify, E.ev[kEvVerify], E.ev[kEvFinalize]);
  hipEventElapsedTime(&st->ms_finalize, E.ev[kEvFinalize], E.ev[kEvEnd]);
  if (has_fs) hipEventElapsedTime(&st->ms_fullscan, E.ev_fs, E.ev[kEvFinalize]);
  hipEventElapsedTime(&st->ms_chunkmap, E.ev[kEvStart], E.ev[kEvK1]);
  hipEventElapsedTime(&st->ms_total, E.ev[kEvStart], E.ev[kEvEnd]);
  hipEventElapsedTime(&st->ms_k0, E.ev_k0[0], E.ev_k0[1]);
}

bool GpuEngine::Enqueue(const uint8_t* d_arena, uint64_t n_bytes, const uint64_t* d_offsets, uint32_t n_files,
                        Ticket* t, std::string* err, FetchOut* fetch, const SkipIn* skip) {
  t->slot = -1;
  if (n_files == 0 || n_bytes >= (uint64_t(1) << 36) - 64 || d_item_diag_ || diag_mode_ != 0) return false;
  int k = -1;
  {
    std::lock_guard<std::mutex> g(slot_mu_);
    for (int i = 0; i < kSlots && k < 0; i++)
      if (!slots_[i].busy) {
        slots_[i].busy = true;
        k = i;
      }
  }
  if (k < 0) return false;
  Slot& S = slots_[k];
  auto fail = [&] {
    (void)hipStreamSynchronize(aux_stream_);
    (void)hipStreamSynchronize(stream_);
    (void)hipStreamSynchronize(rb_stream_);
    if (fetch && fetch_stream_) (void)hipStreamSynchronize(fetch_stream_);
    if (S.lease) GiveFetchBuf(S.lease, S.lease_cap);
    S.lease = nullptr;
    S.lease_cap = 0;
    S.has_fetch = false;
    *err = err_.empty() ? "Enqueue failed" : err_;
    std::lock_guard<std::mutex> g(slot_mu_);
    S.busy = false;
    return false;
  };
  if (hipSetDevice(device_) != hipSuccess) return fail();
  InitCaps(n_bytes);
  if (!S.done) {
    bool ok = hipEventCreateWithFlags(&S.done, hipEventBlockingSync | hipEventDisableTiming) == hipSuccess &&
              S.ev.Create() &&
              hipEventCreateWithFlags(&S.fin, hipEventDisableTiming) == hipSuccess &&
              hipEventCreateWithFlags(&S.rb_done, hipEventDisableTiming) == hipSuccess &&
              hipHostMalloc(reinterpret_cast<void**>(&S.h_cnt), kScanCtrBytes, hipHostMallocDefault) == hipSuccess;
    if (!ok) {
      err_ = "ticket events / pinned counters";
      return fail();
    }
  }
// ... 16 lines not shown
    S.h_cap = caps_.cand;
  }
  uint64_t n_chunks = (n_bytes + kChunk - 1) / kChunk;
  if (n_chunks == 0) n_chunks = 1;
  S.has_fetch = false;
  if (fetch) {
    bool ok = EnsureFetchStream();
    if (ok && !S.h_fctr)
      ok = hipHostMalloc(&S.h_fctr, sizeof(FetchCounters), hipHostMallocDefault) == hipSuccess &&
           hipEventCreate(&S.ev_f[0]) == hipSuccess && hipEventCreate(&S.ev_f[1]) == hipSuccess;
    S.win = fetch->want_windows;
    S.prm = fetch->prm;
    if (ok && S.win) {
      S.stage = fetchw_stage_bytes_.load();
      S.direct = 0;
      const uint64_t rp = fetchw_recent_packed_.load();
      const uint64_t all = FetchGranules(n_bytes) * kFetchGranule;
      const uint64_t copy = std::min(rp + rp / 8 + std::min<uint64_t>(uint64_t(1) << 20, S.stage), all);
      S.fetch_copy = (copy + kFetchGranule - 1) / kFetchGranule * kFetchGranule;
      S.lease = TakeFetchBuf(size_t(S.fetch_copy) + 64, &S.lease_cap);
      ok = S.lease != nullptr;
    } else if (ok) {
      S.stage = fetch_stage_bytes_.load();
      S.direct = fetch_direct_bytes_.load();
      const uint64_t rp = fetch_recent_packed_.load(), rt = fetch_recent_total_.load();
      const uint64_t all = n_bytes + 16 * uint64_t(n_files);
      const uint64_t copy = std::min(rp + rp / 8 + std::min<uint64_t>(uint64_t(1) << 20, S.stage), all);
      S.fetch_copy = (copy + 15) & ~uint64_t(15);
      S.lease = TakeFetchBuf(size_t(std::max(S.fetch_copy, std::min(rt + rt / 8, all)) + 64), &S.lease_cap);
      ok = S.lease != nullptr;
    }
    if (!ok) {
      if (err_.empty()) err_ = "Enqueue: fetch stream / pinned fetch buffer";
      return fail();
    }
  }
  S.has_skip = skip && skip->d_skip && n_bytes > 0;
  if (S.has_skip && !S.h_skip &&
      hipHostMalloc(reinterpret_cast<void**>(&S.h_skip), kScanCtrBytes, hipHostMallocDefault) != hipSuccess) {
    err_ = "pinned skip counters";
    return fail();
  }
  WorkSet& W = sets_[set_turn_];
  set_turn_ = (set_turn_ + 1) % kSets;
  auto enqueue = [&]() -> bool {
    if (!EnqueuePhase(d_arena, n_bytes, d_offsets, n_files, n_chunks, W, overlap_k0_, S.ev, skip)) return false;
    hipStream_t rs = stream_;
    if (readback_stream_) {
      HIP_OK(hipEventRecord(S.fin, stream_));
      HIP_OK(hipStreamWaitEvent(rb_stream_, S.fin, 0));
      rs = rb_stream_;
    }
    HIP_OK(hipMemcpyAsync(S.h_cnt, W.counters, kScanCtrBytes, hipMemcpyDeviceToHost, rs));
    if (S.has_skip) HIP_OK(hipMemcpyAsync(S.h_skip, W.skip_info, kScanCtrBytes, hipMemcpyDeviceToHost, rs));
    HIP_OK(hipMemcpyAsync(S.h_cands, W.cands, size_t(n_copy) * sizeof(Candidate), hipMemcpyDeviceToHost, rs));
    hipStream_t ds = rs;
    if (fetch) {
      if (!(S.win ? IssueFetchWin(W, d_arena, n_bytes, d_offsets, n_files, S.prm, S.stage, S.fetch_copy,
                                  static_cast<uint8_t*>(S.lease), S.h_fctr, S.ev_f[0])
                  : IssueFetch(W, d_arena, d_offsets, n_files, nullptr, S.direct, S.stage, S.fetch_copy,
                               static_cast<uint8_t*>(S.lease), S.h_fctr, S.ev_f[0])))
        return false;
      HIP_OK(hipEventRecord(S.ev_f[1], fetch_stream_));
      if (readback_stream_) {
        HIP_OK(hipEventRecord(S.rb_done, rb_stream_));
        HIP_OK(hipStreamWaitEvent(fetch_stream_, S.rb_done, 0));
      }
      ds = fetch_stream_;
    }
    HIP_OK(hipEventRecord(S.done, ds));
    HIP_OK(hipEventRecord(W.free_ev, ds));
    W.free_rec = true;
    return true;
  };
  if (!enqueue()) {
    if (err_.empty()) err_ = "Enqueue: HIP call failed";
    return fail();
  }
  S.has_fetch = fetch != nullptr;
  S.d_arena = d_arena;
  S.n_bytes = n_bytes;
  S.n_files = n_files;
  S.has_fs = n_fullscan_rules_ > 0;
  t->slot = k;
  t->cand_copy = n_copy;
  return true;
}

bool GpuEngine::Collect(Ticket* t, std::vector<Candidate>* cands, BatchStats* st, bool* rerun, std::string* err,
                        FetchOut* fetch) {
  *rerun = false;
  if (t->slot < 0 || t->slot >= kSlots) {
    *err = "Collect: no ticket";
    return false;
  }
  Slot& S = slots_[t->slot];
  auto release = [&] {
    if (S.lease) GiveFetchBuf(S.lease, S.lease_cap);
    S.lease = nullptr;
    S.lease_cap = 0;
    S.has_fetch = false;
    std::lock_guard<std::mutex> g(slot_mu_);
    S.busy = false;
    t->slot = -1;
  };
  const hipError_t e = WaitEvent(S.done);
  if (e != hipSuccess) {
    *err = std::string("Collect: ") + hipGetErrorString(e);
    release();
    return false;
  }
  BatchStats local;
  if (!st) st = &local;
  *st = BatchStats();
  st->bytes = S.n_bytes;
  st->files = S.n_files;
  const uint32_t* cnt = S.h_cnt;
  const uint32_t n_cands = cnt[kCtCands];
  for (uint32_t seen = cand_recent_.load(); n_cands > seen && !cand_recent_.compare_exchange_weak(seen, n_cands);) {
  }
  if (OverflowedList(cnt) != kListNone || n_cands > t->cand_copy) {
    *rerun = true;
    release();
    return true;
  }
  NoteCounters(cnt, st);
  if (S.has_skip) NoteSkip(S.h_skip, st);
  cands->clear();
  cands->reserve(n_cands);
  for (uint32_t i = 0; i < n_cands; i++)
    if (!(S.h_cands[i].flags & kCandDrop)) cands->push_back(S.h_cands[i]);
  st->candidates = cands->size();
  if (S.has_fetch && S.win) {
    bool ok = fetch != nullptr && fetch->h_offsets != nullptr;
    if (!ok) *err = "Collect: the ticket's scan was enqueued with a fetch";
    if (ok) {
      HostWindowPlan P;
      PlanWindowsOnHost(cands->data(), cands->size(), fetch->h_offsets, S.n_files, h_rule_max_len_.data(),
                        uint32_t(h_rule_max_len_.size()), S.prm, &P);
      const FetchWinCounters& C = *static_cast<const FetchWinCounters*>(S.h_fctr);
      ok = SameWindowPlan(C.granules, C.runs, C.whole_files, P, err);
      if (ok) {
        const uint64_t packed = P.packed_bytes();
        const uint64_t rp = fetchw_recent_packed_.load();
        fetchw_recent_packed_.store(std::max(packed, rp - rp / 8));
        if (packed > S.fetch_copy || packed + 64 > S.lease_cap) {
          *rerun = true;
          release();
          return true;
        }
        float ms = 0;
        if (P.granules) hipEventElapsedTime(&ms, S.ev_f[0], S.ev_f[1]);
        fetch->Release();
        fetch->windows = true;
        fetch->runs = std::move(P.runs);
        fetch->granules = P.granules;
        fetch->whole_marked = P.whole_files;
        fetch->rounds = uint32_t((packed + S.stage - 1) / S.stage);
        fetch->ms_fetch = ms;
        fetch->buf = static_cast<const uint8_t*>(S.lease);
        fetch->owner = this;
        fetch->lease = S.lease;
        fetch->lease_cap = S.lease_cap;
        S.lease = nullptr;
        S.lease_cap = 0;
      }
    }
    if (!ok) {
      release();
      return false;
    }
  } else if (S.has_fetch) {
    bool ok = fetch != nullptr && fetch->h_offsets != nullptr;
    if (!ok) *err = "Collect: the ticket's scan was enqueued with a fetch";
    HostFetchPlan P;
    if (ok) {
      std::vector<uint8_t> want(S.n_files, 0);
      for (const Candidate& c : *cands)
        if (c.file < S.n_files) want[c.file] = 1;
      PlanFetchOnHost(std::move(want), fetch->h_offsets, S.n_files, S.direct, fetch, &P);
      const FetchCounters& C = *static_cast<const FetchCounters*>(S.h_fctr);
      ok = SameFetchPlan(C.packed_bytes, C.n_direct, C.n_files, C.file_bytes, P, err);
    }
    if (ok) {
      NoteFetch(P.packed, P.total);
      if (P.packed > S.fetch_copy || P.total + 64 > S.lease_cap) {
        *rerun = true;
        release();
        return true;
      }
      float ms = 0;
      if (P.files) hipEventElapsedTime(&ms, S.ev_f[0], S.ev_f[1]);
      double ms_direct = 0;
      if (!P.direct.empty()) {
        const auto t0 = std::chrono::steady_clock::now();
        hipError_t e = hipSetDevice(device_);
        for (size_t i = 0; i < P.direct.size() && e == hipSuccess; i++) {
          const uint32_t f = P.direct[i];
          e = hipMemcpyAsync(static_cast<uint8_t*>(S.lease) + fetch->off[f], S.d_arena + fetch->h_offsets[f],
                             size_t(fetch->h_offsets[f + 1] - fetch->h_offsets[f]), hipMemcpyDeviceToHost,
                             fetch_stream_);
        }
        if (e == hipSuccess) e = hipEventRecord(S.ev_f[1], fetch_stream_);
        if (e == hipSuccess) e = WaitEvent(S.ev_f[1]);
        if (e != hipSuccess) {
          *err = std::string("Collect: direct fetch: ") + hipGetErrorString(e);
          ok = false;
        }
// ... 1 lines not shown
      }
      if (ok) {
        FinishFetch(P, S.stage, double(ms) + ms_direct, fetch);
        fetch->buf = static_cast<const uint8_t*>(S.lease);
        fetch->owner = this;
        fetch->lease = S.lease;
        fetch->lease_cap = S.lease_cap;
        S.lease = nullptr;
        S.lease_cap = 0;
      }
    }
    if (!ok) {
      release();
      return false;
    }
  }
  NotePhaseTimes(S.ev, S.has_fs, st);
  release();
  return true;
}

bool GpuEngine::EnsureSets(uint64_t n_chunks, uint32_t n_files, uint64_t f_tiles, bool skip) {
  for (WorkSet& W : sets_) {
    if (skip) {
      if (!Ensure(&W.keep_bits, &W.cap_keep_bits, KeepWords(f_tiles) * 8) ||
          !Ensure(&W.runs, &W.cap_runs, (f_tiles / 2 + 2) * sizeof(uint2)))
        return false;
      if (!W.skip_info) {
        HIP_OK(hipMalloc(reinterpret_cast<void**>(&W.skip_info), kScanCtrBytes));
        HIP_OK(hipMemset(W.skip_info, 0, kScanCtrBytes));
      }
    }
    if (!Ensure(&W.chunk_file, &W.cap_chunk_file, n_chunks * 4) ||
        !Ensure(&W.kw, &W.cap_kw, size_t(n_files) * kw_words_ * 4) ||
        !Ensure(&W.flags, &W.cap_flags, size_t(n_files) * 4) ||
        !Ensure(&W.cands, &W.cap_cands, size_t(caps_.cand) * sizeof(Candidate)))
      return false;
  }
  return true;
}

struct GpuEngine::KernelArgs {
  static FilterParams Filter(const GpuEngine& e, const WorkSet& W, const uint8_t* d_arena, uint64_t n_bytes,
                             const SkipIn* skip) {
    FilterParams fp;
    fp.arena = d_arena;
    fp.n_bytes = n_bytes;
    fp.reach = e.d_reach_;
    fp.diag_mode = e.diag_mode_;
    fp.nl = static_cast<uint16_t*>(e.d_nl_);
    fp.recs = static_cast<uint32_t*>(e.d_recs_);
    fp.rec_cap = e.caps_.rec;
    fp.counters = W.counters;
    fp.runs = skip ? static_cast<const uint2*>(W.runs) : nullptr;
    fp.run_info = skip ? W.skip_info : nullptr;
    return fp;
  }
  static ConfirmParams Confirm(const GpuEngine& e, const WorkSet& W, const uint8_t* d_arena, uint64_t n_bytes,
                               const uint64_t* d_offsets) {
    ConfirmParams cp;
    cp.arena = d_arena;
    cp.n_bytes = n_bytes;
    cp.off = d_offsets;
    cp.chunk_file = static_cast<const uint32_t*>(W.chunk_file);
    cp.nl = static_cast<const uint16_t*>(e.d_nl_);
    cp.reach = e.d_reach_;
    cp.tabs = e.d_ftabs_;
    cp.tabs_bytes = e.ftabs_bytes_;
    cp.t_bucket_off = e.ft_bucket_off_;
    cp.t_bucket_items = e.ft_bucket_items_;
    cp.t_items = e.ft_items_;
    cp.t_item_ids = e.ft_item_ids_;
    cp.t_item_cls = e.ft_item_cls_;
    cp.t_classes = e.ft_classes_;
    cp.anchors = e.d_anchors_;
    cp.rules = e.d_rules_;
    cp.nfa = e.d_nfa_;
    cp.recs = static_cast<const uint32_t*>(e.d_recs_);
    cp.rec_cap = e.caps_.rec;
    cp.flags = static_cast<uint32_t*>(W.flags);
    cp.counters = W.counters;
    cp.hits = static_cast<uint32_t*>(e.d_hits_);
    cp.hit_cap = e.caps_.hit;
    cp.folds = static_cast<FoldSite*>(e.d_folds_);
    cp.fold_cap = e.caps_.fold;
    cp.diag = e.diag_confirm_;
    cp.kwbits = static_cast<uint32_t*>(W.kw);
    cp.kw_words = e.kw_words_;
    cp.core = e.d_core_;
    cp.group_items = e.d_group_items_;
    cp.bucket_groups = e.d_bucket_groups_;
    cp.item_diag = e.d_item_diag_;
    cp.t_luts = e.ft_luts_;
    cp.t_cmap = e.ft_cmap_;
    cp.t_ccore = e.ft_ccore_;
    cp.t_gitems = e.ft_gitems_;
    cp.t_bgroups = e.ft_bgroups_;
    cp.n_cls = e.n_core_cls_;
    cp.t_hkeys = e.ft_hkeys_;
    cp.t_hitems = e.ft_hitems_;
    cp.hash_bits = e.hash_bits_;
    cp.hash_buckets = e.hash_buckets_;
    cp.n_classes_lds = e.c_stage_classes_ ? e.n_fclasses_ : 0u;
    return cp;
  }
  static FoldParams Fold(const GpuEngine& e, const WorkSet& W, const uint8_t* d_arena, const uint64_t* d_offsets) {
    FoldParams fo;
    fo.arena = d_arena;
    fo.off = d_offsets;
    fo.tabs = e.d_ftabs_;
    fo.tabs_bytes = e.ftabs_fold_bytes_;
    fo.t_items = e.ft_items_;
    fo.t_item_ids = e.ft_item_ids_;
    fo.t_item_cls = e.ft_item_cls_;
    fo.t_classes = e.ft_classes_;
    fo.n_items = e.n_fitems_;
    fo.stage_items = e.fold_stage_ ? 1u : 0u;
    fo.n_classes = e.n_fclasses_;
    static const uint32_t fold_diag =
        std::getenv("TSG_DIAG_FOLD") ? uint32_t(std::atoi(std::getenv("TSG_DIAG_FOLD"))) : 0u;
    fo.diag = fold_diag;
    fo.pairs = static_cast<const FoldPair*>(e.d_fold_pairs_);
    fo.first = static_cast<const uint32_t*>(e.d_fold_first_);
    fo.n_pairs_k = e.n_fold_pairs_k_;
    fo.n_pairs_s = e.n_fold_pairs_s_;
    fo.n_cap_k = e.n_fold_cap_k_;
    fo.n_cap_s = e.n_fold_cap_s_;
    fo.folds = static_cast<const FoldSite*>(e.d_folds_);
    fo.fold_cap = e.caps_.fold;
    fo.idx_off = static_cast<const uint32_t*>(e.d_fold_idx_off_);
    fo.idx_items = static_cast<const uint32_t*>(e.d_fold_idx_items_);
    fo.n_cap_k_idx = e.n_fold_cap_k_idx_;
    fo.n_cap_s_idx = e.n_fold_cap_s_idx_;
    fo.hits = static_cast<uint32_t*>(e.d_hits_);
    fo.hit_cap = e.caps_.hit;
    fo.counters = W.counters;
    return fo;
  }
  static KwFoldParams KwFold(const GpuEngine& e, const WorkSet& W, const uint8_t* d_arena,
                             const uint64_t* d_offsets) {
    KwFoldParams kf;
    kf.arena = d_arena;
    kf.off = d_offsets;
    kf.tabs = static_cast<const uint8_t*>(e.d_ftabs_);
    kf.t_items = e.ft_items_;
    kf.t_item_ids = e.ft_item_ids_;
    kf.t_item_cls = e.ft_item_cls_;
    kf.t_classes = e.ft_classes_;
    kf.pairs = static_cast<const FoldPair*>(e.d_kwfold_pairs_);
    kf.n_rng_i = e.n_kwf_ri_;
    kf.n_rng_k = e.n_kwf_rk_;
    kf.n_cap_i = e.n_kwf_ci_;
    kf.n_cap_k = e.n_kwf_ck_;
    kf.folds = static_cast<const FoldSite*>(e.d_folds_);
    kf.fold_cap = e.caps_.fold;
    kf.counters = W.counters;
    kf.kwbits = static_cast<uint32_t*>(W.kw);
    kf.kw_words = e.kw_words_;
    return kf;
  }
  static NfaParams Nfa(const GpuEngine& e, const WorkSet& W, const uint8_t* d_arena, const uint64_t* d_offsets,
                       uint32_t n_files, const SkipIn* skip) {
    NfaParams np;
    np.arena = d_arena;
    np.off = d_offsets;
    np.n_files = n_files;
    np.nl = static_cast<const uint16_t*>(e.d_nl_);
    np.anchors = e.d_anchors_;
    np.rules = e.d_rules_;
    np.rule_kw = e.d_rule_kw_;
    np.kwbits = static_cast<const uint32_t*>(W.kw);
    np.kw_words = e.kw_words_;
    np.flags = static_cast<const uint32_t*>(W.flags);
    np.nfa = e.d_nfa_;
    np.hits = static_cast<const uint32_t*>(e.d_hits_);
    np.hit_cap = e.caps_.hit;
    np.counters = W.counters;
    static const uint32_t verify_diag =
        std::getenv("TSG_DIAG_VERIFY") ? uint32_t(std::atoi(std::getenv("TSG_DIAG_VERIFY"))) : 0u;
    np.diag = verify_diag;
    np.cands = static_cast<Candidate*>(W.cands);
    np.cand_cap = e.caps_.cand;
    np.fullscan_rules = e.d_fullscan_rules_;
    np.n_fullscan_rules = e.n_fullscan_rules_;
    np.fs_chunk = e.fs_chunk_;
    np.skip = skip ? skip->d_skip : nullptr;
    np.drop_marked = skip && skip->drop_marked ? 1u : 0u;
    np.kw_fold = e.kw_fold_ ? 1u : 0u;
    return np;
  }
  static FsLists FullScanLists(const GpuEngine& e, const WorkSet& W) {
    FsLists fq;
    fq.pairs = static_cast<FsPair*>(e.d_fs_pairs_);
    fq.pair_cap = e.caps_.fs_pair;
    fq.tasks = static_cast<FsTask*>(e.d_fs_tasks_);
    fq.task_cap = e.caps_.fs_task;
    fq.wave_pairs = static_cast<uint32_t*>(e.d_fs_wave_);
    fq.ctr = W.fs_ctr;
    fq.task_min = e.caps_.fs_task_bytes;
    return fq;
  }
};

bool GpuEngine::EnqueuePhase(const uint8_t* d_arena, uint64_t n_bytes, const uint64_t* d_offsets, uint32_t n_files,
                             uint64_t n_chunks, WorkSet& W, bool k0_aux, PhaseEvents& E, const SkipIn* skip) {
  const uint64_t f_tiles = (n_bytes + kFTile - 1) / kFTile;
  if (skip && (!skip->d_skip || f_tiles == 0)) skip = nullptr;
  if (!EnsureSets(n_chunks, n_files, f_tiles, skip != nullptr)) return false;
  if (!Ensure(&d_nl_, &cap_nl_, (n_chunks + 8) * 2) ||
      !Ensure(&d_folds_, &cap_folds_, size_t(caps_.fold) * sizeof(FoldSite)) ||
      !Ensure(&d_recs_, &cap_recs_, size_t(caps_.rec) * 4) ||
      !Ensure(&d_hits_, &cap_hits_, size_t(caps_.hit) * 12))
    return false;
  if (n_fullscan_rules_ > 0 &&
      (!Ensure(&d_fs_pairs_, &cap_fs_pairs_, size_t(caps_.fs_pair) * sizeof(FsPair)) ||
       !Ensure(&d_fs_wave_, &cap_fs_wave_, size_t(caps_.fs_pair) * 4) ||
       !Ensure(&d_fs_tasks_, &cap_fs_tasks_, size_t(caps_.fs_task) * 4 * sizeof(FsTask))))
    return false;
  const hipStream_t k0s = k0_aux ? aux_stream_ : stream_;
  if (skip && skip->ready) HIP_OK(hipStreamWaitEvent(k0s, skip->ready, 0));
  if (W.free_rec) HIP_OK(hipStreamWaitEvent(k0s, W.free_ev, 0));
  if (!k0_aux && W.k0_rec) HIP_OK(hipStreamWaitEvent(stream_, W.k0_done, 0));
  if (k0_aux && k2_rec_) HIP_OK(hipStreamWaitEvent(aux_stream_, k2_done_, 0));
  if (!k0_aux) {
    HIP_OK(hipEventRecord(E.ev[kEvStart], stream_));
    if (d_item_diag_) HIP_OK(hipMemsetAsync(d_item_diag_, 0, 8 * std::max<size_t>(n_fitems_, 1), stream_));
  }
  HIP_OK(hipEventRecord(E.ev_k0[0], k0s));
  {
    const uint64_t used = (n_bytes + kChunk - 1) / kChunk;
    const uint64_t runs = (used + kK0Run - 1) / kK0Run;
    const uint64_t clear_q = (uint64_t(n_files) * (1 + kw_words_) + 3) / 4;
    const uint64_t work = std::max(runs, clear_q);
    const uint32_t blocks = uint32_t(std::max<uint64_t>(1, std::min<uint64_t>((work + 255) / 256, 8192)));
    ClearParams z;
    z.flags = static_cast<uint32_t*>(W.flags);
    z.kw = static_cast<uint32_t*>(W.kw);
    z.n_kw = uint64_t(n_files) * kw_words_;
    z.counters = W.counters;
    z.fs_ctr = n_fullscan_rules_ > 0 ? W.fs_ctr : nullptr;
    z.skip_info = skip ? W.skip_info : nullptr;
    chunk_map_kernel<<<blocks, 256, 0, k0s>>>(d_offsets, n_files, used, static_cast<uint32_t*>(W.chunk_file), z);
    HIP_OK(hipGetLastError());
  }
  if (skip) {
    const uint32_t blocks =
        uint32_t(std::max<uint64_t>(1, std::min<uint64_t>((KeepWords(f_tiles) * 64 + 255) / 256, 4096)));
    tile_keep_kernel<<<blocks, 256, 0, k0s>>>(d_offsets, n_files, static_cast<const uint32_t*>(W.chunk_file),
                                              skip->d_skip, n_bytes, f_tiles, static_cast<uint64_t*>(W.keep_bits),
                                              W.skip_info);
    HIP_OK(hipGetLastError());
    tile_runs_kernel<<<1, kRunThreads, 0, k0s>>>(static_cast<const uint64_t*>(W.keep_bits), f_tiles,
                                                 static_cast<uint2*>(W.runs), W.skip_info);
    HIP_OK(hipGetLastError());
  }
  HIP_OK(hipEventRecord(E.ev_k0[1], k0s));
  if (k0_aux) {
    HIP_OK(hipEventRecord(W.k0_done, aux_stream_));
    W.k0_rec = true;
    HIP_OK(hipEventRecord(E.ev[kEvStart], stream_));
    if (d_item_diag_) HIP_OK(hipMemsetAsync(d_item_diag_, 0, 8 * std::max<size_t>(n_fitems_, 1), stream_));
    HIP_OK(hipStreamWaitEvent(stream_, W.k0_done, 0));
  }
  const FilterParams fp = KernelArgs::Filter(*this, W, d_arena, n_bytes, skip);
  uint32_t f_grid =
      uint32_t(std::max<uint64_t>(1, std::min<uint64_t>((f_tiles + kScanWaves - 1) / kScanWaves, 256 * kFWgPerCu)));
  if (k1_grid_cap_) f_grid = std::min(f_grid, k1_grid_cap_);
  HIP_OK(hipEventRecord(E.ev[kEvK1], stream_));
  if (skip) filter_kernel<true><<<f_grid, kScanThreads, 0, stream_>>>(fp);
  else filter_kernel<false><<<f_grid, kScanThreads, 0, stream_>>>(fp);
  HIP_OK(hipGetLastError());
  HIP_OK(hipEventRecord(E.ev[kEvK2], stream_));
  const ConfirmParams cp = KernelArgs::Confirm(*this, W, d_arena, n_bytes, d_offsets);
  if (diag_mode_ == 0) {
    if (lds_tabs_)
      confirm_kernel<true><<<2048 * 256 / kCThreads, kCThreads, c_lds_bytes_, stream_>>>(cp);
    else
      confirm_kernel<false><<<2048 * 256 / kCThreadsG, kCThreadsG, c_lds_bytes_, stream_>>>(cp);
  }
  HIP_OK(hipGetLastError());
  HIP_OK(hipEventRecord(E.ev[kEvFold], stream_));
  HIP_OK(hipEventRecord(k2_done_, stream_));
  k2_rec_ = true;
  const FoldParams fo = KernelArgs::Fold(*this, W, d_arena, d_offsets);
  if (diag_mode_ == 0) {
    if (lds_tabs_)
      fold_kernel<true><<<fold_grid_, 64 * kFoldWaves, ftabs_fold_bytes_ + 32 * n_fitems_, stream_>>>(fo);
    else if (fold_stage_)
      fold_kernel<false, 16><<<2048, 64 * 16, fold_stage_bytes_, stream_>>>(fo);
    else
      fold_kernel<false><<<2048, 64 * kFoldWaves, 0, stream_>>>(fo);
  }
  HIP_OK(hipGetLastError());
  if (diag_mode_ == 0 && kw_fold_ && n_kwf_ci_ + n_kwf_ck_ > 0) {
    const KwFoldParams kf = KernelArgs::KwFold(*this, W, d_arena, d_offsets);
    kwfold_kernel<<<1024, 64 * kFoldWaves, 0, stream_>>>(kf);
    HIP_OK(hipGetLastError());
  }
  HIP_OK(hipEventRecord(E.ev[kEvVerify], stream_));
  const NfaParams np = KernelArgs::Nfa(*this, W, d_arena, d_offsets, n_files, skip);
  if (diag_mode_ == 0) verify_hits_kernel<<<verify_blocks_, 256, 0, stream_>>>(np);
  HIP_OK(hipGetLastError());
  if (np.n_fullscan_rules > 0) {
    HIP_OK(hipEventRecord(E.ev_fs, stream_));
    const FsLists fq = KernelArgs::FullScanLists(*this, W);
    const uint64_t pairs = uint64_t(n_files) * n_fullscan_rules_;
    const uint32_t pb = uint32_t(std::min<uint64_t>(std::max<uint64_t>((pairs + 255) / 256, 1), 4096));
    fs_pairs_kernel<<<pb, 256, 0, stream_>>>(np, fq);
    HIP_OK(hipGetLastError());
    fs_task_kernel<<<2048, 256, 0, stream_>>>(np, fq);
    HIP_OK(hipGetLastError());
    fs_wave_kernel<<<1024, 256, 0, stream_>>>(np, fq);
    HIP_OK(hipGetLastError());
  }
  HIP_OK(hipEventRecord(E.ev[kEvFinalize], stream_));
  if (diag_mode_ == 0) finalize_kernel<<<finalize_blocks_, 256, 0, stream_>>>(np);
  HIP_OK(hipGetLastError());
  HIP_OK(hipEventRecord(E.ev[kEvEnd], stream_));
  return true;
}


void FetchOut::Release() {
  if (owner && lease) owner->GiveFetchBuf(lease, lease_cap);
  owner = nullptr;
  lease = nullptr;
  lease_cap = 0;
  buf = nullptr;
}

void GpuEngine::SetFetchSizes(uint64_t stage_bytes, uint64_t direct_bytes) {
  fetch_stage_bytes_.store(std::max<uint64_t>(kFetchSeg, stage_bytes / kFetchSeg * kFetchSeg));
  fetch_direct_bytes_.store(std::max<uint64_t>(1, direct_bytes));
  fetchw_stage_bytes_.store(std::max<uint64_t>(kFetchGranule, stage_bytes / kFetchGranule * kFetchGranule));
}

void* GpuEngine::TakeFetchBuf(size_t need, size_t* cap) { return fetch_pool_->Take(need, cap); }
void GpuEngine::GiveFetchBuf(void* p, size_t cap) { fetch_pool_->Give(p, cap); }

bool GpuEngine::EnsureFetchStream() {
  if (fetch_stream_) return true;
  HIP_OK(hipStreamCreateWithFlags(&fetch_stream_, hipStreamNonBlocking));
  HIP_OK(hipEventCreateWithFlags(&ev_packed_, hipEventDisableTiming));
  HIP_OK(hipEventCreateWithFlags(&ev_drained_, hipEventDisableTiming));
  HIP_OK(hipEventCreate(&ev_run_f_[0]));
  HIP_OK(hipEventCreate(&ev_run_f_[1]));
  HIP_OK(hipMalloc(&d_fctr_, sizeof(FetchCounters)));
  HIP_OK(hipHostMalloc(&h_run_fctr_, sizeof(FetchCounters), hipHostMallocDefault));
  return true;
}

void GpuEngine::NoteFetch(uint64_t packed, uint64_t total) {
  const uint64_t rp = fetch_recent_packed_.load(), rt = fetch_recent_total_.load();
  fetch_recent_packed_.store(std::max(packed, rp - rp / 8));
  fetch_recent_total_.store(std::max(total, rt - rt / 8));
}

bool GpuEngine::IssueFetch(const WorkSet& W, const uint8_t* d_arena, const uint64_t* d_offsets, uint32_t n_files,
                           const uint32_t* h_flags, uint64_t direct, uint64_t stage, uint64_t copy_bytes,
                           uint8_t* h_dst, void* h_ctr, hipEvent_t ev0) {
  if (!EnsureFetchStream()) return false;
// ... 156 lines not shown
  }
  float ms = 0;
  hipEventElapsedTime(&ms, ev_run_f_[0], ev_run_f_[1]);
  out->runs = std::move(P.runs);
  out->granules = P.granules;
  out->whole_marked = P.whole_files;
  out->rounds = uint32_t((packed + stage - 1) / stage);
  out->ms_fetch = ms;
  return true;
}

bool GpuEngine::FetchFiles(const uint8_t* d_arena, const uint64_t* d_offsets, uint32_t n_files,
                           const std::vector<uint8_t>& want, FetchOut* out) {
  HIP_OK(hipSetDevice(device_));
  const WorkSet& W = sets_[0];
  if (W.free_rec) HIP_OK(hipStreamWaitEvent(stream_, W.free_ev, 0));
  if (W.k0_rec) HIP_OK(hipStreamWaitEvent(stream_, W.k0_done, 0));
  return FetchNow(d_arena, d_offsets, n_files, want, true, out);
}

bool GpuEngine::DumpStages(const WorkSet& W, const uint32_t* cnt, uint64_t n_bytes, uint32_t n_files, StageDump* d) {
  std::memcpy(d->counters, cnt, sizeof(d->counters));
  d->kw_words = kw_words_;
  d->hit_cap = caps_.hit;
  d->rec_cap = caps_.rec;
  d->cand_cap = caps_.cand;
  const uint64_t used = (n_bytes + kChunk - 1) / kChunk;
  const size_t n_hits = std::min(cnt[kCtHits], caps_.hit), n_recs = std::min(cnt[kCtRecs], caps_.rec);
  std::vector<uint32_t> raw(3 * n_hits);
  d->kw.assign(size_t(n_files) * kw_words_, 0);
  d->flags.assign(n_files, 0);
  d->nl.assign(used, 0);
  d->recs.assign(n_recs, 0);
  d->chunk_file.assign(used, 0);
  auto get = [&](void* dst, const void* src, size_t bytes) {
    return bytes == 0 || hipMemcpy(dst, src, bytes, hipMemcpyDeviceToHost) == hipSuccess;
  };
  if (!get(raw.data(), d_hits_, raw.size() * 4) || !get(d->kw.data(), W.kw, d->kw.size() * 4) ||
      !get(d->flags.data(), W.flags, d->flags.size() * 4) || !get(d->nl.data(), d_nl_, d->nl.size() * 2) ||
      !get(d->recs.data(), d_recs_, d->recs.size() * 4) ||
      !get(d->chunk_file.data(), W.chunk_file, d->chunk_file.size() * 4)) {
    err_ = "stage dump: device to host copy failed";
    return false;
  }
  d->hits.resize(n_hits);
  for (size_t i = 0; i < n_hits; i++) hit_unpack(&raw[3 * i], &d->hits[i].file, &d->hits[i].end, &d->hits[i].aid);
  return true;
}

bool GpuEngine::Run(const uint8_t* d_arena, uint64_t n_bytes, const uint64_t* d_offsets, uint32_t n_files,
                    std::vector<Candidate>* cands, BatchStats* st, FetchOut* fetch, const SkipIn* skip,
                    StageDump* dump) {
  HIP_OK(hipSetDevice(device_));
  cands->clear();
  BatchStats local;
  if (!st) st = &local;
  *st = BatchStats();
  st->bytes = n_bytes;
  st->files = n_files;
  if (n_files == 0) return true;
  if (n_bytes >= (uint64_t(1) << 36) - 64) {
    err_ = "batch arena must be < 64 GiB";
    return false;
  }
  uint64_t n_chunks = (n_bytes + kChunk - 1) / kChunk;
  if (n_chunks == 0) n_chunks = 1;
  InitCaps(n_bytes);
  WorkSet& W = sets_[0];
  for (int attempt = 0; attempt < 8; attempt++) {
    if (!EnqueuePhase(d_arena, n_bytes, d_offsets, n_files, n_chunks, W, false, run_ev_, skip)) return false;
    uint32_t cnt[kScanCtrWords];
    if (!h_run_cnt_) HIP_OK(hipHostMalloc(reinterpret_cast<void**>(&h_run_cnt_), sizeof(cnt), hipHostMallocDefault));
    HIP_OK(hipMemcpyAsync(h_run_cnt_, W.counters, sizeof(cnt), hipMemcpyDeviceToHost, stream_));
    const bool has_skip = skip && skip->d_skip && n_bytes > 0;
    if (has_skip) {
      if (!h_run_skip_)
        HIP_OK(hipHostMalloc(reinterpret_cast<void**>(&h_run_skip_), kScanCtrBytes, hipHostMallocDefault));
      HIP_OK(hipMemcpyAsync(h_run_skip_, W.skip_info, kScanCtrBytes, hipMemcpyDeviceToHost, stream_));
    }
    HIP_OK(WaitStream());
    if (has_skip) NoteSkip(h_run_skip_, st);
    std::memcpy(cnt, h_run_cnt_, sizeof(cnt));
    if (std::getenv("TSG_STATS_DEBUG"))
      std::fprintf(stderr, "counters: hits %u cands %u special %u recs %u folds %u\n", cnt[kCtHits], cnt[kCtCands],
                   cnt[kCtSpecial], cnt[kCtRecs], cnt[kCtFolds]);
    NoteCounters(cnt, st);
    uint32_t fc[kScanCtrWords] = {};
    if (OverflowedList(cnt) == kListFullScan) HIP_OK(hipMemcpy(fc, W.fs_ctr, sizeof(fc), hipMemcpyDeviceToHost));
    if (GrowOverflowed(cnt, fc, &caps_) != kListNone) continue;
    const uint32_t n_cands = cnt[kCtCands];
    cands->resize(n_cands);
    if (n_cands) {
      const size_t nb = size_t(n_cands) * sizeof(Candidate);
      if (!EnsureHost(&h_run_cands_, &cap_h_run_cands_, nb)) return false;
      HIP_OK(hipMemcpyAsync(h_run_cands_, W.cands, nb, hipMemcpyDeviceToHost, stream_));
      HIP_OK(WaitStream());
      std::memcpy(cands->data(), h_run_cands_, nb);
    }
    if (dump) {
      dump->cands = *cands;
      if (!DumpStages(W, cnt, n_bytes, n_files, dump)) return false;
    }
    cands->erase(std::remove_if(cands->begin(), cands->end(), [](const Candidate& c) { return c.flags & kCandDrop; }),
                 cands->end());
    st->candidates = cands->size();
    if (d_item_diag_) DumpItemDiag();
    NotePhaseTimes(run_ev_, n_fullscan_rules_ > 0, st);
    if (fetch) {
      std::vector<uint8_t> want(n_files, 0);
      for (const Candidate& c : *cands)
        if (c.file < n_files) want[c.file] = 1;
      if (fetch->want_windows) {
        if (!FetchNowWin(d_arena, n_bytes, d_offsets, n_files, *cands, fetch)) return false;
      } else if (!FetchNow(d_arena, d_offsets, n_files, std::move(want), false, fetch)) {
        return false;
      }
    }
    return true;
  }
  err_ = "candidate buffers kept overflowing";
  return false;
}

void GpuEngine::NoteSkip(const uint32_t* info, BatchStats* st) const {
  st->skip_runs = info[kSkRuns];
  st->tiles = info[kSkTiles];
  st->skip_tiles = info[kSkTiles] - info[kSkKept];
  st->skip_files = info[kSkFiles];
  st->skip_bytes = uint64_t(info[kSkBytes]) | (uint64_t(info[kSkBytes + 1]) << 32);
  st->skip_wave_runs = info[kSkWaveRuns];
}

void GpuEngine::DumpItemDiag() {
  std::vector<uint32_t> v(2 * std::max<size_t>(n_fitems_, 1));
  if (hipMemcpy(v.data(), d_item_diag_, v.size() * 4, hipMemcpyDeviceToHost) != hipSuccess) return;
  FILE* fp = std::fopen(item_diag_path_.c_str(), "a");
  if (!fp) return;
  for (uint32_t i = 0; i < n_fitems_; i++)
    std::fprintf(fp, "%u %u %u %u %u\n", i, uint32_t(h_items_kind_[i]), h_items_id_[i], v[2 * i], v[2 * i + 1]);
  std::fprintf(fp, "--\n");
  std::fclose(fp);
}

}
```

trivy_amd/csrc/scan_layout.h:

```cpp
#pragma once
#include <algorithm>
#include <cstddef>
#include <cstdint>

namespace tsg {

constexpr uint32_t kScanCtrWords = 16;
constexpr size_t kScanCtrBytes = kScanCtrWords * sizeof(uint32_t);

constexpr uint32_t kCtHits = 0,
                   kCtCands = 1,
                   kCtSpecial = 2,
                   kCtHitOvf = 3,
                   kCtCandOvf = 4,
                   kCtUnused5 = 5,
                   kCtFsOvf = 6,
                   kCtRecs = 7,
                   kCtRecOvf = 8,
                   kCtFolds = 9,
                   kCtFoldOvf = 10,
                   kCtAnchorHits = 11,
                   kCtUnused12 = 12,
                   kCtOpenPairs = 13,
                   kCtUnused14 = 14, kCtUnused15 = 15;

constexpr uint32_t kFsPairs = 0,
                   kFsTasks = 1,
                   kFsWidths = 4,
                   kFsWavePairs = 5,
                   kNFsCtr = 6;

constexpr uint32_t kSkRuns = 0,
                   kSkKept = 1,
                   kSkTailKept = 2,
                   kSkFiles = 3,
                   kSkBytes = 4,
                   kSkWaveRuns = 6,
                   kSkTiles = 7;

enum : int {
  kEvStart = 0,
  kEvK1 = 1,
  kEvK2 = 2,
  kEvFold = 3,
  kEvVerify = 4,
  kEvFinalize = 5,
  kEvEnd = 6,
  kNScanEv = 7
};

struct ScanCaps {
  uint32_t hit = 0, cand = 0, rec = 0, fold = 0;
  uint32_t fs_pair = 0, fs_task = 0;
  uint32_t fs_task_bytes = 4096;
};

constexpr uint32_t kFsTaskRecBytes = 8;
constexpr uint64_t kMaxFsTasks = 0x7FFFFFFFu / kFsTaskRecBytes / kFsWidths;

enum ScanList { kListNone = 0, kListRecs, kListFullScan, kListFolds, kListHits, kListCands };

inline ScanList OverflowedList(const uint32_t* cnt) {
  if (cnt[kCtRecOvf]) return kListRecs;
  if (cnt[kCtFsOvf]) return kListFullScan;
  if (cnt[kCtFoldOvf]) return kListFolds;
  if (cnt[kCtHitOvf]) return kListHits;
  if (cnt[kCtCandOvf]) return kListCands;
  return kListNone;
}

inline ScanList GrowOverflowed(const uint32_t* cnt, const uint32_t* fc, ScanCaps* c) {
  auto grown = [](uint32_t n, uint32_t slack, uint32_t rec_bytes) {
    return uint32_t(std::min<uint64_t>(uint64_t(n) + n / 4 + slack, 0xFFFFFFF0u / rec_bytes));
  };
  const ScanList which = OverflowedList(cnt);
  switch (which) {
    case kListNone: break;
    case kListRecs: c->rec = grown(cnt[kCtRecs], 4096, 4); break;
    case kListFullScan: {
      c->fs_pair = std::max<uint32_t>(c->fs_pair, fc[kFsPairs] + fc[kFsPairs] / 4 + 1024);
      uint32_t mt = 0;
      for (uint32_t w = 0; w < kFsWidths; w++) mt = std::max(mt, fc[kFsTasks + w]);
      const uint64_t want = uint64_t(mt) + mt / 4 + 1024;
      if (want > kMaxFsTasks) {
        uint64_t tb = c->fs_task_bytes;
        while (tb < (uint64_t(1) << 26) && want * c->fs_task_bytes / tb > kMaxFsTasks) tb *= 2;
        c->fs_task_bytes = uint32_t(tb);
      }
      c->fs_task = uint32_t(std::min<uint64_t>(std::max<uint64_t>(c->fs_task, want), kMaxFsTasks));
      break;
    }
    case kListFolds: c->fold = grown(cnt[kCtFolds], 1024, 16); break;
    case kListHits: c->hit = grown(cnt[kCtHits], 1024, 12); break;
    case kListCands: c->cand = grown(cnt[kCtCands], 1024, 1); break;
  }
  return which;
}

}
```

Before: 3146.

## Split confirm kernel into class-check match stage and separate emit kernel

The confirm kernel now only runs the per-byte class-set check and writes compact 8-byte (start, item) match records through a per-wave LDS buffer. A new emit_kernel reads those records and does the file lookup, keyword bits, fold sites, follow-LUT checks and hit emission. The aim is to take the divergent, register-heavy tail out of the confirm loop, which should improve its occupancy and uniformity. The cost is an extra kernel launch, a global match buffer sized from the input with its own overflow and rerun path, and one more round trip through memory. There are also small tweaks to fire_e indexing and follow_words loading to keep the arrays in registers.

New measurement: 3253, median of 6. +3.4%, better.

```diff
diff --git a/include/tsg_debug.h b/include/tsg_debug.h
--- a/include/tsg_debug.h
+++ b/include/tsg_debug.h
@@ -58,6 +58,7 @@
 
 struct tsg_scanner;
 int tsg_debug_scanner_engine(struct tsg_scanner* s, uint64_t out[4]);
+int tsg_debug_scanner_match_cap(struct tsg_scanner* s, uint64_t* cap);
 int tsg_debug_filter_orform(const tsg_compiled* c, uint32_t out[1024]);
 
 int tsg_debug_scanner_gpu_findings(struct tsg_scanner* s, int mode);
@@ -109,6 +110,8 @@
                                  const uint64_t* offsets, uint32_t n_files, const uint8_t tail[64],
                                  const uint8_t* skip, tsg_debug_stage_dump* out);
 int tsg_debug_scan_grow(const uint32_t counters[16], const uint32_t fs_counters[6], uint32_t caps[7]);
+int tsg_debug_scan_grow_matches(const uint32_t counters[16], const uint32_t fs_counters[6], uint32_t caps[8]);
+void tsg_debug_match_record(uint64_t start, uint32_t item, uint32_t words[2], uint64_t* start_out, uint32_t* item_out);
 
 int tsg_debug_tar_headers(int device, const void* dev_tar, uint64_t n_bytes, uint64_t capacity, uint32_t grid_cap,
                           void* records_out, uint64_t* count_out, double* ms_out);
diff --git a/trivy_amd/csrc/capi_debug.cpp b/trivy_amd/csrc/capi_debug.cpp
--- a/trivy_amd/csrc/capi_debug.cpp
+++ b/trivy_amd/csrc/capi_debug.cpp
@@ -545,9 +545,24 @@
   tsg::ScanCaps c;
   uint32_t* const field[7] = {&c.hit, &c.cand, &c.rec, &c.fold, &c.fs_pair, &c.fs_task, &c.fs_task_bytes};
   for (int i = 0; i < 7; i++) *field[i] = caps[i];
+  c.match = 0xFFFFFFFFu;
   const int which = tsg::GrowOverflowed(counters, fs_counters, &c);
   for (int i = 0; i < 7; i++) caps[i] = *field[i];
   return which;
+}
+
+int tsg_debug_scan_grow_matches(const uint32_t* counters, const uint32_t* fs_counters, uint32_t caps[8]) {
+  tsg::ScanCaps c;
+  uint32_t* const field[8] = {&c.hit, &c.cand, &c.rec, &c.fold, &c.fs_pair, &c.fs_task, &c.fs_task_bytes, &c.match};
+  for (int i = 0; i < 8; i++) *field[i] = caps[i];
+  const int which = tsg::GrowOverflowed(counters, fs_counters, &c);
+  for (int i = 0; i < 8; i++) caps[i] = *field[i];
+  return which;
+}
+
+void tsg_debug_match_record(uint64_t start, uint32_t item, uint32_t words[2], uint64_t* start_out, uint32_t* item_out) {
+  tsg::match_pack(start, item, words);
+  tsg::match_unpack(words, start_out, item_out);
 }
 
 int tsg_debug_pool_budget(void) { return tsg::PoolBudget(); }
diff --git a/trivy_amd/csrc/capi_scanner.cpp b/trivy_amd/csrc/capi_scanner.cpp
--- a/trivy_amd/csrc/capi_scanner.cpp
+++ b/trivy_amd/csrc/capi_scanner.cpp
@@ -706,6 +706,14 @@
   return 0;
 }
 
+int tsg_debug_scanner_match_cap(tsg_scanner* s, uint64_t* cap) {
+  *cap = 0;
+  if (!s || !s->s || s->s->n_engines() == 0) return -1;
+  for (size_t i = 0; i < s->s->n_engines(); i++)
+    *cap = std::max<uint64_t>(*cap, s->s->engine_at(i)->host_mem_info().match_cap);
+  return 0;
+}
+
 int tsg_scanner_set_fetch_options(tsg_scanner* s, const tsg_fetch_options* opt) {
   if (!s || !s->s || !opt) {
     tsg::SetError("tsg_scanner_set_fetch_options: NULL argument");
diff --git a/trivy_amd/csrc/engine.h b/trivy_amd/csrc/engine.h
--- a/trivy_amd/csrc/engine.h
+++ b/trivy_amd/csrc/engine.h
@@ -189,6 +189,7 @@
     Candidate* h_cands = nullptr;
     size_t h_cap = 0;
     bool busy = false, has_fs = false;
+    uint32_t match_cap = 0;
     uint64_t n_bytes = 0;
     uint32_t n_files = 0;
     bool has_fetch = false;
@@ -246,6 +247,7 @@
  public:
   struct HostMemInfo {
     uint64_t retired_pending, retired_freed, cand_cap, slot_bytes;
+    uint64_t match_cap;
   };
   HostMemInfo host_mem_info();
 
@@ -302,6 +304,7 @@
   uint32_t k1_grid_cap_ = 0;
   void NoteSkip(const uint32_t* info, BatchStats* st) const;
   void* d_hits_ = nullptr; size_t cap_hits_ = 0;
+  void* d_matches_ = nullptr; size_t cap_matches_ = 0;
   void* d_folds_ = nullptr; size_t cap_folds_ = 0;
   hipStream_t copy_stream_ = nullptr;
   static constexpr int kNStage = 4;
@@ -351,6 +354,7 @@
   hipEvent_t ev_sync_ = nullptr;
   bool blocking_sync_ = true;
   uint32_t verify_blocks_ = 4096;
+  uint32_t emit_blocks_ = 1024;
   uint32_t finalize_blocks_ = 16384;
   hipError_t WaitStream();
   hipError_t WaitEvent(hipEvent_t ev);
diff --git a/trivy_amd/csrc/engine.hip b/trivy_amd/csrc/engine.hip
--- a/trivy_amd/csrc/engine.hip
+++ b/trivy_amd/csrc/engine.hip
@@ -728,6 +728,51 @@
   wave_sync();
 }
 
+#ifndef TSG_C_MATCHES
+#define TSG_C_MATCHES 128
+#endif
+constexpr uint32_t kCWaveMatches = TSG_C_MATCHES;
+constexpr uint32_t kCMatchFlush = kCWaveMatches / 2;
+static_assert(kCMatchFlush >= 64, "a wave stages up to 64 matches between two flush checks");
+
+__device__ __forceinline__ void stage_match(uint32_t* mbuf, uint32_t* mcnt, uint32_t* matches, uint32_t cap,
+                                            uint32_t* counters, uint64_t start, uint32_t item) {
+  uint32_t w[2];
+  match_pack(start, item, w);
+  const uint32_t k = atomicAdd(mcnt, 1u);
+  if (k < kCWaveMatches) {
+    mbuf[2 * k + 0] = w[0];
+    mbuf[2 * k + 1] = w[1];
+    return;
+  }
+  const uint32_t g = atomicAdd(&counters[kCtMatches], 1u);
+  if (g < cap) {
+    matches[2ull * g + 0] = w[0];
+    matches[2ull * g + 1] = w[1];
+  }
+}
+
+__device__ __forceinline__ void flush_matches(uint32_t* mbuf, uint32_t* mcnt, uint32_t* matches, uint32_t cap,
+                                              uint32_t* counters, uint32_t lane) {
+  wave_sync();
+  const uint32_t n_all = __builtin_amdgcn_readfirstlane(*mcnt);
+  const uint32_t n = n_all < kCWaveMatches ? n_all : kCWaveMatches;
+  if (n) {
+    uint32_t base = 0;
+    if (lane == 0) base = atomicAdd(&counters[kCtMatches], n);
+    base = __builtin_amdgcn_readfirstlane(base);
+    for (uint32_t i = lane; i < n; i += 64) {
+      if (base + i < cap) {
+        matches[2ull * (base + i) + 0] = mbuf[2 * i + 0];
+        matches[2ull * (base + i) + 1] = mbuf[2 * i + 1];
+      }
+    }
+  }
+  wave_sync();
+  if (lane == 0) *mcnt = 0;
+  wave_sync();
+}
+
 __device__ __forceinline__ void put_hit(uint32_t* hits, uint32_t cap, uint32_t* counters, uint32_t f, uint64_t end,
                                         uint32_t aid) {
   const uint32_t g = wave_slot(&counters[kCtHits]);
@@ -789,8 +834,7 @@
 
 __device__ __forceinline__ void follow_words(const uint32_t* w, uint32_t s, uint32_t* X) {
   uint32_t R[14];
-#pragma unroll
-  for (int j = 0; j < 14; j++) R[j] = w[j];
+  __builtin_memcpy(R, w, sizeof(R));
 #pragma unroll
   for (int j = 0; j < 13; j++) X[j] = __builtin_amdgcn_alignbyte(R[j + 1], R[j], s & 3);
 }
@@ -820,6 +864,8 @@
   uint32_t hit_cap;
   FoldSite* folds;
   uint32_t fold_cap;
+  uint32_t* matches;
+  uint32_t match_cap;
   uint32_t diag;
   uint32_t* kwbits;
   uint32_t kw_words;
@@ -956,7 +1002,7 @@
 constexpr uint32_t kCQ2 = TSG_C_Q2;
 constexpr size_t ConfirmFixedLds(int t) {
   return 4096 + size_t(t) * (kCWin + 8) + size_t(t / 64) * (kCQ1 + kCQ2) * 4 +
-         size_t(t / 64) * kCWaveHits * 12 + size_t(t / 64) * 16;
+         size_t(t / 64) * kCWaveMatches * kMatchRecBytes + size_t(t / 64) * 16;
 }
 
 template <bool kLdsTabs>
@@ -972,8 +1018,8 @@
   uint64_t* s_base = reinterpret_cast<uint64_t*>(s_win + kCThreads * kCWin);
   uint32_t* s_q1 = reinterpret_cast<uint32_t*>(s_base + kCThreads);
   uint32_t* s_q2 = s_q1 + kWaves * kCQ1;
-  uint32_t* s_hbuf = s_q2 + kWaves * kCQ2;
-  uint32_t* s_cnt = s_hbuf + kWaves * kCWaveHits * 3;
+  uint32_t* s_mbuf = s_q2 + kWaves * kCQ2;
+  uint32_t* s_cnt = s_mbuf + kWaves * kCWaveMatches * 2;
   uint8_t* s_tabs = reinterpret_cast<uint8_t*>(s_cnt + kWaves * 4);
   const int tid = threadIdx.x;
   load_reach_lds(s_reach, P.reach, tid, blockDim.x);
@@ -1001,9 +1047,8 @@
   uint64_t* wbase = s_base + wave * 64;
   uint32_t* q1 = s_q1 + wave * kCQ1;
   uint32_t* q2 = s_q2 + wave * kCQ2;
-  uint32_t* hbuf = s_hbuf + wave * kCWaveHits * 3;
+  uint32_t* mbuf = s_mbuf + wave * kCWaveMatches * 2;
   const uint32_t n_recs = P.counters[kCtRecs] < P.rec_cap ? P.counters[kCtRecs] : P.rec_cap;
-  uint32_t n_anchor = 0;
   auto check_item = [&](uint32_t l, uint32_t k, uint32_t ix, uint32_t full) {
     const FilterItemGpu it = items[ix];
     const uint64_t base = wbase[l];
@@ -1012,66 +1057,14 @@
     const uint32_t core_lo = full ? uint32_t(it.back) : (it.back > 8 ? it.back - 8u : 0u);
     const uint64_t cw0 = base >= 16 ? base - 16 : 0;
     const uint8_t* cwin = wwin + l * kCWin;
-    auto sets_ok = [&](uint32_t q0, uint32_t q1) {
-      for (uint32_t q = q0; q < q1; q++) {
-        if (q >= core_lo && q < it.back) continue;
-        const uint64_t pos = uint64_t(start) + q;
-        const uint32_t bt = pos - cw0 < uint64_t(kCWin) ? uint32_t(cwin[pos - cw0]) : uint32_t(P.arena[pos]);
-        const uint32_t c = item_cls[it.cls_off + q];
-        if (!((classes[c * 8 + (bt >> 5)] >> (bt & 31)) & 1u)) return false;
-      }
-      return true;
-    };
-    const uint32_t check_to = it.lit_end < it.n && (P.diag & 32) ? it.lit_end : it.n;
-    if (!sets_ok(0, check_to)) return;
-    if (P.diag & 16) return;
-    const uint64_t s0 = uint64_t(start);
-    uint32_t f = P.chunk_file[s0 / kChunk];
-    uint64_t fs = P.off[f], fe = P.off[f + 1];
-    while (s0 >= fe) {
-      f++;
-      fs = fe;
-      fe = P.off[f + 1];
-    }
-    if (s0 < fs || s0 + it.n > fe) return;
-    if (P.diag & 8) return;
-    if (it.kind == kItemKeyword) {
-      const uint32_t id = item_ids[it.ids_off];
-      uint32_t* w = &P.kwbits[uint64_t(f) * P.kw_words + (id >> 5)];
-      const uint32_t bit = 1u << (id & 31);
-      if (!(__hip_atomic_load(w, __ATOMIC_RELAXED, __HIP_MEMORY_SCOPE_AGENT) & bit)) atomicOr(w, bit);
-      return;
-    }
-    if (it.kind == kItemFold) {
-      const uint32_t fl = item_ids[it.ids_off] == 2 ? 3u : 5u;
-      if (atomicOr(&P.flags[f], fl) == 0) atomicAdd(&P.counters[kCtSpecial], 1u);
-      const uint32_t q = atomicAdd(&P.counters[kCtFolds], 1u);
-      if (q < P.fold_cap) P.folds[q] = FoldSite{s0, f, it.n};
-      else P.counters[kCtFoldOvf] = 1;
-      return;
-    }
-    if (P.item_diag) atomicAdd(&P.item_diag[2 * ix], 1u);
-    const uint64_t lit_end = (s0 - fs) + it.lit_end;
-    const uint64_t e = s0 + it.lit_end;
-    const uint64_t w0 = wbase[l] >= 16 ? wbase[l] - 16 : 0;
-    uint32_t X[13];
-    bool have_x = false;
-    int after = check_to < it.n ? -1 : 1;
-    for (uint32_t d = 0; d < it.n_ids; d++) {
-      const uint32_t aid = item_ids[it.ids_off + d];
-      n_anchor++;
-      const FollowLut lut = reinterpret_cast<const FollowLut*>(tabs + P.t_luts)[aid];
-      if (lut.n[0] && e < P.n_bytes) {
-        if (!have_x) {
-          follow_words(reinterpret_cast<const uint32_t*>(P.arena + (e & ~uint64_t(3))), uint32_t(e), X);
-          have_x = true;
-        }
-        if (!follow_lut_pass(lut, X, int64_t(fe - e))) continue;
-      }
-      if (after < 0) after = sets_ok(check_to, it.n) ? 1 : 0;
-      if (!after) return;
-      stage_hit(hbuf, &cnt[0], P.hits, P.hit_cap, P.counters, f, lit_end, aid);
-    }
+    for (uint32_t q = 0; q < it.n; q++) {
+      if (q >= core_lo && q < it.back) continue;
+      const uint64_t pos = uint64_t(start) + q;
+      const uint32_t bt = pos - cw0 < uint64_t(kCWin) ? uint32_t(cwin[pos - cw0]) : uint32_t(P.arena[pos]);
+      const uint32_t c = item_cls[it.cls_off + q];
+      if (!((classes[c * 8 + (bt >> 5)] >> (bt & 31)) & 1u)) return;
+    }
+    stage_match(mbuf, &cnt[0], P.matches, P.match_cap, P.counters, uint64_t(start), ix);
   };
   auto run_q2 = [&]() {
     wave_sync();
@@ -1082,7 +1075,7 @@
         const uint32_t e = q2[c2 + lane];
         check_item(e & 63u, (e >> 6) & 15u, (e >> 10) & 0x1FFFFFu, e >> 31);
       }
-      if (__builtin_amdgcn_readfirstlane(cnt[0]) >= 64) flush_staged(hbuf, &cnt[0], P.hits, P.hit_cap, P.counters, lane);
+      if (__builtin_amdgcn_readfirstlane(cnt[0]) >= kCMatchFlush) flush_matches(mbuf, &cnt[0], P.matches, P.match_cap, P.counters, lane);
     }
     wave_sync();
     if (lane == 0) cnt[2] = 0;
@@ -1168,7 +1161,7 @@
     rec_next = rec_nn;
     load_win(rec_next, r + stride < n_recs, dwn);
     rec_nn = r + 2 * stride < n_recs ? P.recs[r + 2 * stride] : 0u;
-    uint32_t fire_e[4], n_fire = 0;
+    uint32_t fire_e[4] = {0, 0, 0, 0}, n_fire = 0;
     if (r < n_recs) {
       const uint64_t base = uint64_t(rec) * 16;
       const uint4 d0 = dw[0], d1 = dw[1];
@@ -1193,8 +1186,10 @@
 #pragma unroll
           for (int w = 0; w < kFWords; w++) fm |= ((~st[w] >> 20) & 0xFu) << (4 * w);
           const uint32_t fe = lane | (k << 6) | (fm << 10);
-          if (n_fire < 4) fire_e[n_fire] = fe;
-          else do_fire(fe);
+#pragma unroll
+          for (uint32_t s = 0; s < 4; s++)
+            if (n_fire == s) fire_e[s] = fe;
+          if (n_fire >= 4) do_fire(fe);
           n_fire++;
         }
       }
@@ -1208,7 +1203,9 @@
         if (lane >= uint32_t(x)) incl += t;
       }
       const uint32_t at = __builtin_amdgcn_readfirstlane(cnt[1]) + incl - mine;
-      for (uint32_t i = 0; i < mine; i++) {
+#pragma unroll
+      for (uint32_t i = 0; i < 4; i++) {
+        if (i >= mine) continue;
         if (at + i < kCQ1) q1[at + i] = fire_e[i];
         else do_fire(fire_e[i]);
       }
@@ -1225,13 +1222,153 @@
     }
     wave_sync();
     if (lane == 0) cnt[1] = 0;
-    if (__builtin_amdgcn_readfirstlane(cnt[0]) >= 64) flush_staged(hbuf, &cnt[0], P.hits, P.hit_cap, P.counters, lane);
+    if (__builtin_amdgcn_readfirstlane(cnt[0]) >= kCMatchFlush) flush_matches(mbuf, &cnt[0], P.matches, P.match_cap, P.counters, lane);
     wave_sync();
   }
-  flush_staged(hbuf, &cnt[0], P.hits, P.hit_cap, P.counters, lane);
-#pragma unroll
-  for (int x = 32; x >= 1; x >>= 1) n_anchor += __shfl_xor(n_anchor, x);
-  if (lane == 0 && n_anchor) atomicAdd(&P.counters[kCtAnchorHits], n_anchor);
+  flush_matches(mbuf, &cnt[0], P.matches, P.match_cap, P.counters, lane);
+}
+
+constexpr int kEmitThreads = 256;
+constexpr uint32_t kEmitFolds = 96;
+
+__device__ __forceinline__ void stage_fold(FoldSite* fbuf, uint32_t* fcnt, FoldSite* folds, uint32_t cap,
+                                           uint32_t* counters, const FoldSite& site) {
+  const uint32_t k = atomicAdd(fcnt, 1u);
+  if (k < kEmitFolds) {
+    fbuf[k] = site;
+    return;
+  }
+  const uint32_t q = atomicAdd(&counters[kCtFolds], 1u);
+  if (q < cap) folds[q] = site;
+  else counters[kCtFoldOvf] = 1;
+}
+
+__device__ __forceinline__ void flush_folds(FoldSite* fbuf, uint32_t* fcnt, FoldSite* folds, uint32_t cap,
+                                            uint32_t* counters, uint32_t lane) {
+  wave_sync();
+  const uint32_t n_all = __builtin_amdgcn_readfirstlane(*fcnt);
+  const uint32_t n = n_all < kEmitFolds ? n_all : kEmitFolds;
+  if (n) {
+    uint32_t base = 0;
+    if (lane == 0) base = atomicAdd(&counters[kCtFolds], n);
+    base = __builtin_amdgcn_readfirstlane(base);
+    for (uint32_t i = lane; i < n; i += 64) {
+      if (base + i < cap) folds[base + i] = fbuf[i];
+      else counters[kCtFoldOvf] = 1;
+    }
+  }
+  wave_sync();
+  if (lane == 0) *fcnt = 0;
+  wave_sync();
+}
+
+#ifndef TSG_E_MINW
+#define TSG_E_MINW 4
+#endif
+__global__ __launch_bounds__(kEmitThreads, TSG_E_MINW) void emit_kernel(ConfirmParams P) {
+  constexpr uint32_t kWaves = kEmitThreads / 64;
+  __shared__ uint32_t s_hbuf[kWaves * kCWaveHits * 3];
+  __shared__ FoldSite s_fbuf[kWaves * kEmitFolds];
+  __shared__ uint32_t s_cnt[kWaves], s_fcnt[kWaves], s_sum[2];
+  const uint32_t tid = threadIdx.x, lane = tid & 63, wave = tid >> 6;
+  uint32_t* hbuf = s_hbuf + wave * kCWaveHits * 3;
+  FoldSite* fbuf = s_fbuf + wave * kEmitFolds;
+  uint32_t* cnt = s_cnt + wave;
+  uint32_t* fcnt = s_fcnt + wave;
+  if (lane == 0) *cnt = *fcnt = 0;
+  if (tid < 2) s_sum[tid] = 0;
+  __syncthreads();
+  const uint8_t* tabs = static_cast<const uint8_t*>(P.tabs);
+  const FilterItemGpu* items = reinterpret_cast<const FilterItemGpu*>(tabs + P.t_items);
+  const uint32_t* item_ids = reinterpret_cast<const uint32_t*>(tabs + P.t_item_ids);
+  const FollowLut* luts = reinterpret_cast<const FollowLut*>(tabs + P.t_luts);
+  const uint32_t n_all = P.counters[kCtMatches];
+  const uint32_t n = n_all < P.match_cap ? n_all : P.match_cap;
+  uint32_t n_anchor = 0, n_special = 0;
+  auto emit_one = [&](uint64_t s0, uint32_t ix) {
+    if (P.diag & 16) return;
+    typedef uint32_t ItemWords __attribute__((ext_vector_type(4), aligned(4)));
+    static_assert(sizeof(FilterItemGpu) == 16 && offsetof(FilterItemGpu, n) == 0 && offsetof(FilterItemGpu, lit_end) == 4 &&
+                      offsetof(FilterItemGpu, kind) == 6 && offsetof(FilterItemGpu, n_ids) == 7 &&
+                      offsetof(FilterItemGpu, ids_off) == 8,
+                  "FilterItemGpu layout");
+    const ItemWords iw = *reinterpret_cast<const ItemWords*>(items + ix);
+    struct {
+      uint32_t n, lit_end, kind, n_ids, ids_off;
+    } const it = {iw.x & 0xFFFFu, iw.y & 0xFFFFu, (iw.y >> 16) & 0xFFu, iw.y >> 24, iw.z};
+    uint32_t f = P.chunk_file[s0 / kChunk];
+    const bool anchor = it.kind != kItemKeyword && it.kind != kItemFold;
+    const uint64_t e = s0 + it.lit_end;
+    const bool have_x = anchor && e < P.n_bytes;
+    uint32_t X[13];
+    if (have_x) {
+      follow_words(reinterpret_cast<const uint32_t*>(P.arena + (e & ~uint64_t(3))), uint32_t(e), X);
+    } else {
+#pragma unroll
+      for (int j = 0; j < 13; j++) X[j] = 0;
+    }
+    uint64_t fs = P.off[f], fe = P.off[f + 1];
+    while (s0 >= fe) {
+      f++;
+      fs = fe;
+      fe = P.off[f + 1];
+    }
+    if (s0 < fs || s0 + it.n > fe) return;
+    if (P.diag & 8) return;
+    if (it.kind == kItemKeyword) {
+      const uint32_t id = item_ids[it.ids_off];
+      uint32_t* w = &P.kwbits[uint64_t(f) * P.kw_words + (id >> 5)];
+      const uint32_t bit = 1u << (id & 31);
+      if (!(__hip_atomic_load(w, __ATOMIC_RELAXED, __HIP_MEMORY_SCOPE_AGENT) & bit)) atomicOr(w, bit);
+      return;
+    }
+    if (it.kind == kItemFold) {
+      const uint32_t fl = item_ids[it.ids_off] == 2 ? 3u : 5u;
+      if (atomicOr(&P.flags[f], fl) == 0) n_special++;
+      stage_fold(fbuf, fcnt, P.folds, P.fold_cap, P.counters, FoldSite{s0, f, it.n});
+      return;
+    }
+    if (P.item_diag) atomicAdd(&P.item_diag[2 * ix], 1u);
+    const uint64_t lit_end = (s0 - fs) + it.lit_end;
+    for (uint32_t d = 0; d < it.n_ids; d++) {
+      const uint32_t aid = item_ids[it.ids_off + d];
+      n_anchor++;
+      typedef uint32_t LutWords __attribute__((ext_vector_type(8), aligned(4)));
+      const LutWords lw = *reinterpret_cast<const LutWords*>(luts + aid);
+      FollowLut lut;
+      __builtin_memcpy(&lut, &lw, sizeof(lut));
+      if (lut.n[0] && have_x && !follow_lut_pass(lut, X, int64_t(fe - e))) continue;
+      stage_hit(hbuf, cnt, P.hits, P.hit_cap, P.counters, f, lit_end, aid);
+    }
+  };
+  const uint64_t stride = uint64_t(gridDim.x) * kEmitThreads;
+  for (uint64_t i0 = uint64_t(blockIdx.x) * kEmitThreads + wave * 64; i0 < n; i0 += stride) {
+    const uint64_t i = i0 + lane;
+    if (i < n) {
+      const uint2 m = reinterpret_cast<const uint2*>(P.matches)[i];
+      const uint32_t w[2] = {m.x, m.y};
+      uint64_t s0;
+      uint32_t ix;
+      match_unpack(w, &s0, &ix);
+      emit_one(s0, ix);
+    }
+    if (__builtin_amdgcn_readfirstlane(*cnt) >= 64) flush_staged(hbuf, cnt, P.hits, P.hit_cap, P.counters, lane);
+    if (__builtin_amdgcn_readfirstlane(*fcnt) >= 32) flush_folds(fbuf, fcnt, P.folds, P.fold_cap, P.counters, lane);
+  }
+  flush_staged(hbuf, cnt, P.hits, P.hit_cap, P.counters, lane);
+  flush_folds(fbuf, fcnt, P.folds, P.fold_cap, P.counters, lane);
+#pragma unroll
+  for (int x = 32; x >= 1; x >>= 1) {
+    n_anchor += __shfl_xor(n_anchor, x);
+    n_special += __shfl_xor(n_special, x);
+  }
+  if (lane == 0) {
+    if (n_anchor) atomicAdd(&s_sum[0], n_anchor);
+    if (n_special) atomicAdd(&s_sum[1], n_special);
+  }
+  __syncthreads();
+  if (tid == 0 && s_sum[0]) atomicAdd(&P.counters[kCtAnchorHits], s_sum[0]);
+  if (tid == 1 && s_sum[1]) atomicAdd(&P.counters[kCtSpecial], s_sum[1]);
 }
 
 struct FoldPair {
@@ -2156,6 +2293,7 @@
   hipEventCreateWithFlags(&ev_sync_, hipEventBlockingSync | hipEventDisableTiming);
   if (const char* bs = std::getenv("TSG_BLOCKING_SYNC")) blocking_sync_ = std::atoi(bs) != 0;
   if (const char* vb = std::getenv("TSG_VERIFY_BLOCKS")) verify_blocks_ = uint32_t(std::max(1, std::atoi(vb)));
+  if (const char* eb = std::getenv("TSG_EMIT_BLOCKS")) emit_blocks_ = uint32_t(std::max(1, std::atoi(eb)));
   if (const char* fb = std::getenv("TSG_FINALIZE_BLOCKS")) finalize_blocks_ = uint32_t(std::max(1, std::atoi(fb)));
   kw_words_ = std::max<uint32_t>(1, cr.kw_words());
   n_rules_ = uint32_t(cr.rules.size());
@@ -2453,7 +2591,7 @@
   hipSetDevice(device_);
   void* ps[] = {d_item_diag_, d_fold_pairs_, d_kwfold_pairs_, d_fold_idx_off_, d_fold_idx_items_, d_fold_first_, d_reach_, d_core_, d_group_items_, d_bucket_groups_, d_ftabs_, d_folds_, d_recs_, d_anchors_,
                 d_rules_, d_rule_kw_, d_nfa_, d_fullscan_rules_, d_nl_,
-                d_hits_, d_fs_pairs_, d_fs_tasks_, d_fs_wave_, d_xlen_, d_xoff_, d_xscan_,
+                d_hits_, d_matches_, d_fs_pairs_, d_fs_tasks_, d_fs_wave_, d_xlen_, d_xoff_, d_xscan_,
                 d_xf_, d_gfiles_, d_gdst_, d_gbuf_};
   for (void* p : ps)
     if (p) hipFree(p);
@@ -2574,7 +2712,7 @@
 }
 
 GpuEngine::HostMemInfo GpuEngine::host_mem_info() {
-  HostMemInfo m{retired_pending_.load(), retired_freed_.load(), caps_.cand, 0};
+  HostMemInfo m{retired_pending_.load(), retired_freed_.load(), caps_.cand, 0, caps_.match};
   std::lock_guard<std::mutex> g(slot_mu_);
   for (const auto& S : slots_) m.slot_bytes += uint64_t(S.h_cap) * sizeof(Candidate);
   return m;
@@ -3012,6 +3150,7 @@
   if (caps_.cand == 0) caps_.cand = 1 << 16;
   if (caps_.rec == 0) caps_.rec = uint32_t(std::min<uint64_t>(std::max<uint64_t>(n_bytes / 128, 1 << 16), 1u << 30));
   if (caps_.fold == 0) caps_.fold = 1 << 16;
+  if (caps_.match == 0) caps_.match = uint32_t(std::min<uint64_t>(std::max<uint64_t>(n_bytes / 512, 1 << 16), 1u << 28));
   if (caps_.fs_pair == 0) caps_.fs_pair = 1 << 14;
   if (caps_.fs_task == 0) caps_.fs_task = 1 << 16;
 }
@@ -3194,6 +3333,7 @@
   S.n_bytes = n_bytes;
   S.n_files = n_files;
   S.has_fs = n_fullscan_rules_ > 0;
+  S.match_cap = caps_.match;
   t->slot = k;
   t->cand_copy = n_copy;
   return true;
@@ -3231,11 +3371,14 @@
   const uint32_t n_cands = cnt[kCtCands];
   for (uint32_t seen = cand_recent_.load(); n_cands > seen && !cand_recent_.compare_exchange_weak(seen, n_cands);) {
   }
-  if (OverflowedList(cnt) != kListNone || n_cands > t->cand_copy) {
+  if (OverflowedList(cnt, S.match_cap) != kListNone || n_cands > t->cand_copy) {
     *rerun = true;
     release();
     return true;
   }
+  if (std::getenv("TSG_STATS_DEBUG"))
+    std::fprintf(stderr, "collected: hits %u cands %u recs %u folds %u matches %u (capacity %u)\n", cnt[kCtHits],
+                 cnt[kCtCands], cnt[kCtRecs], cnt[kCtFolds], cnt[kCtMatches], S.match_cap);
   NoteCounters(cnt, st);
   if (S.has_skip) NoteSkip(S.h_skip, st);
   cands->clear();
@@ -3403,6 +3546,8 @@
     cp.counters = W.counters;
     cp.hits = static_cast<uint32_t*>(e.d_hits_);
     cp.hit_cap = e.caps_.hit;
+    cp.matches = static_cast<uint32_t*>(e.d_matches_);
+    cp.match_cap = e.caps_.match;
     cp.folds = static_cast<FoldSite*>(e.d_folds_);
     cp.fold_cap = e.caps_.fold;
     cp.diag = e.diag_confirm_;
@@ -3531,7 +3676,8 @@
   if (!Ensure(&d_nl_, &cap_nl_, (n_chunks + 8) * 2) ||
       !Ensure(&d_folds_, &cap_folds_, size_t(caps_.fold) * sizeof(FoldSite)) ||
       !Ensure(&d_recs_, &cap_recs_, size_t(caps_.rec) * 4) ||
-      !Ensure(&d_hits_, &cap_hits_, size_t(caps_.hit) * 12))
+      !Ensure(&d_hits_, &cap_hits_, size_t(caps_.hit) * 12) ||
+      !Ensure(&d_matches_, &cap_matches_, size_t(caps_.match) * kMatchRecBytes))
     return false;
   if (n_fullscan_rules_ > 0 &&
       (!Ensure(&d_fs_pairs_, &cap_fs_pairs_, size_t(caps_.fs_pair) * sizeof(FsPair)) ||
@@ -3598,6 +3744,8 @@
       confirm_kernel<true><<<2048 * 256 / kCThreads, kCThreads, c_lds_bytes_, stream_>>>(cp);
     else
       confirm_kernel<false><<<2048 * 256 / kCThreadsG, kCThreadsG, c_lds_bytes_, stream_>>>(cp);
+    HIP_OK(hipGetLastError());
+    emit_kernel<<<emit_blocks_, kEmitThreads, 0, stream_>>>(cp);
   }
   HIP_OK(hipGetLastError());
   HIP_OK(hipEventRecord(E.ev[kEvFold], stream_));
@@ -3920,11 +4068,12 @@
     if (has_skip) NoteSkip(h_run_skip_, st);
     std::memcpy(cnt, h_run_cnt_, sizeof(cnt));
     if (std::getenv("TSG_STATS_DEBUG"))
-      std::fprintf(stderr, "counters: hits %u cands %u special %u recs %u folds %u\n", cnt[kCtHits], cnt[kCtCands],
-                   cnt[kCtSpecial], cnt[kCtRecs], cnt[kCtFolds]);
+      std::fprintf(stderr, "counters: hits %u cands %u special %u recs %u folds %u matches %u (capacity %u)\n",
+                   cnt[kCtHits], cnt[kCtCands], cnt[kCtSpecial], cnt[kCtRecs], cnt[kCtFolds], cnt[kCtMatches],
+                   caps_.match);
     NoteCounters(cnt, st);
     uint32_t fc[kScanCtrWords] = {};
-    if (OverflowedList(cnt) == kListFullScan) HIP_OK(hipMemcpy(fc, W.fs_ctr, sizeof(fc), hipMemcpyDeviceToHost));
+    if (OverflowedList(cnt, caps_.match) == kListFullScan) HIP_OK(hipMemcpy(fc, W.fs_ctr, sizeof(fc), hipMemcpyDeviceToHost));
     if (GrowOverflowed(cnt, fc, &caps_) != kListNone) continue;
     const uint32_t n_cands = cnt[kCtCands];
     cands->resize(n_cands);
diff --git a/trivy_amd/csrc/scan_layout.h b/trivy_amd/csrc/scan_layout.h
--- a/trivy_amd/csrc/scan_layout.h
+++ b/trivy_amd/csrc/scan_layout.h
@@ -20,7 +20,7 @@
                    kCtFolds = 9,
                    kCtFoldOvf = 10,
                    kCtAnchorHits = 11,
-                   kCtUnused12 = 12,
+                   kCtMatches = 12,
                    kCtOpenPairs = 13,
                    kCtUnused14 = 14, kCtUnused15 = 15;
 
@@ -51,6 +51,7 @@
 
 struct ScanCaps {
   uint32_t hit = 0, cand = 0, rec = 0, fold = 0;
+  uint32_t match = 0;
   uint32_t fs_pair = 0, fs_task = 0;
   uint32_t fs_task_bytes = 4096;
 };
@@ -58,10 +59,27 @@
 constexpr uint32_t kFsTaskRecBytes = 8;
 constexpr uint64_t kMaxFsTasks = 0x7FFFFFFFu / kFsTaskRecBytes / kFsWidths;
 
-enum ScanList { kListNone = 0, kListRecs, kListFullScan, kListFolds, kListHits, kListCands };
+enum ScanList { kListNone = 0, kListRecs, kListFullScan, kListFolds, kListHits, kListCands, kListMatches };
 
-inline ScanList OverflowedList(const uint32_t* cnt) {
+#if defined(__HIPCC__)
+#define TSG_HOST_DEVICE __host__ __device__
+#else
+#define TSG_HOST_DEVICE
+#endif
+constexpr uint32_t kMatchStartBits = 36, kMatchItemBits = 21, kMatchRecBytes = 8;
+static_assert(kMatchStartBits > 32 && kMatchStartBits - 32 + kMatchItemBits <= 32, "a match record is two words");
+TSG_HOST_DEVICE inline void match_pack(uint64_t start, uint32_t item, uint32_t* w) {
+  w[0] = uint32_t(start);
+  w[1] = (uint32_t(start >> 32) & ((1u << (kMatchStartBits - 32)) - 1u)) | (item << (kMatchStartBits - 32));
+}
+TSG_HOST_DEVICE inline void match_unpack(const uint32_t* w, uint64_t* start, uint32_t* item) {
+  *start = uint64_t(w[0]) | (uint64_t(w[1] & ((1u << (kMatchStartBits - 32)) - 1u)) << 32);
+  *item = (w[1] >> (kMatchStartBits - 32)) & ((1u << kMatchItemBits) - 1u);
+}
+
+inline ScanList OverflowedList(const uint32_t* cnt, uint32_t match_cap) {
   if (cnt[kCtRecOvf]) return kListRecs;
+  if (cnt[kCtMatches] > match_cap) return kListMatches;
   if (cnt[kCtFsOvf]) return kListFullScan;
   if (cnt[kCtFoldOvf]) return kListFolds;
   if (cnt[kCtHitOvf]) return kListHits;
@@ -73,10 +91,11 @@
   auto grown = [](uint32_t n, uint32_t slack, uint32_t rec_bytes) {
     return uint32_t(std::min<uint64_t>(uint64_t(n) + n / 4 + slack, 0xFFFFFFF0u / rec_bytes));
   };
-  const ScanList which = OverflowedList(cnt);
+  const ScanList which = OverflowedList(cnt, c->match);
   switch (which) {
     case kListNone: break;
     case kListRecs: c->rec = grown(cnt[kCtRecs], 4096, 4); break;
+    case kListMatches: c->match = grown(cnt[kCtMatches], 1024, kMatchRecBytes); break;
     case kListFullScan: {
       c->fs_pair = std::max<uint32_t>(c->fs_pair, fc[kFsPairs] + fc[kFsPairs] / 4 + 1024);
       uint32_t mt = 0;
```
